# matthiasverstraete/3d_recognizer

Measured on AMD Instinct MI355X. Metric: training clouds/sec, N=40960 pts, bs=8, at 1/2/4/8 GPUs; mIoU parity, higher is better.
Workload: dtype f32 storage/accumulate, bf16x3 MFMA in the wide GEMMs

## Files before the change

### 3d_recognizer_amd/csrc/gemm.hip

```cpp
#include "rl_common.h"
#include <stdlib.h>
#include <string.h>

namespace {

typedef float f32x4 __attribute__((ext_vector_type(4)));

constexpr int GM_BM = 128;
constexpr int GM_BK = 16;
constexpr int GM_AS = 20;

struct AOperand {
    const float* A;
    long lda, a_bstride;
    int a_mode;
    RlLazy lazy;
    const float* xyz;
    long xyz_bstride;
    const int32_t* nbr_idx;
    const float* nbr_d2;
    int nbr_k;
    int n;
    int K;
    long M;
// ... 17 lines not shown
            const long R = row0 + r;
            float v[10];
#pragma unroll
            for (int c = 0; c < 10; ++c) v[c] = 0.f;
            if (R < row_limit) {
                const long p = (unsigned)R / (unsigned)a.nbr_k;
                const int b = (int)((unsigned)p / (unsigned)a.n);
                const int i = (int)(p - (long)b * a.n);
                const int j = a.nbr_idx[R];
                const float* xb = a.xyz + (long)b * a.xyz_bstride * 3;
                const float xi = xb[(long)i * 3 + 0], yi = xb[(long)i * 3 + 1], zi = xb[(long)i * 3 + 2];
                const float xj = xb[(long)j * 3 + 0], yj = xb[(long)j * 3 + 1], zj = xb[(long)j * 3 + 2];
                v[0] = xi; v[1] = yi; v[2] = zi;
                v[3] = xj; v[4] = yj; v[5] = zj;
                v[6] = xi - xj; v[7] = yi - yj; v[8] = zi - zj;
                v[9] = __fsqrt_rn(a.nbr_d2[R]);
            }
            float* dst = As + r * stride;
#pragma unroll
            for (int c = 0; c < 10; ++c) dst[c] = v[c];
            for (int c = 10; c < kw; ++c) dst[c] = 0.f;
        }
        return;
    }
    if (a.vec4) {
        const int qpr = kw >> 2;
        for (int e = tid; e < nrows * qpr; e += 256) {
            const int r = e / qpr, q = e - r * qpr;
            const long R = row0 + r;
            const int kc = k0 + q * 4;
            float4 v = make_float4(0.f, 0.f, 0.f, 0.f);
            if (R < row_limit && kc < a.K) {
                v = *reinterpret_cast<const float4*>(a.A + a_row_offset(a, R) + kc);
                if (a.lazy.scale) {
                    v.x = rl_lazy(a.lazy, v.x, kc + 0);
                    v.y = rl_lazy(a.lazy, v.y, kc + 1);
                    v.z = rl_lazy(a.lazy, v.z, kc + 2);
                    v.w = rl_lazy(a.lazy, v.w, kc + 3);
                }
            }
            *reinterpret_cast<float4*>(As + r * stride + q * 4) = v;
        }
        return;
    }
    for (int e = tid; e < nrows * kw; e += 256) {
        const int r = e / kw, c = e - r * kw;
        const long R = row0 + r;
        const int kc = k0 + c;
        float v = 0.f;
        if (R < row_limit && kc < a.K) v = rl_lazy(a.lazy, a.A[a_row_offset(a, R) + kc], kc);
        As[r * stride + c] = v;
    }
}

struct GemmParams {
    AOperand a;
    int N;
    const float* W;
    long w_ks, w_ns;
    const float* bias;
    float* Y;
    long ldy, y_bstride;
    int rows_per_batch;
    int y_contig;
    int accumulate;
    double* stats;
    const float* piv_mean;
    const float* piv_bias;
    int ksplit;
    int kchunk;
    float* kslab;
    int stat_slots;
    int gx, ny;
    const float* addend;
    float* out2;
    const int32_t* out2_index;
    long out2_bstride;
    int split_col;
    const __bf16* wsplit;
    const float* bnb_Y;
    const float* bnb_scale;
    const float* bnb_shift;
    const float* bnb_mean;
    const float* bnb_invstd;
    float bnb_neg;
    int pair_ny1;
    int N2;
    float* Y2;
    double* stats2;
    const float* piv_mean2;
    const float* piv_bias2;
    const __bf16* wsplit2;
};

__device__ __forceinline__ float stat_pivot(const GemmParams& p, int c) {
    if (!p.stats || !p.piv_mean || c >= p.N) return 0.f;
    return p.piv_mean[c] - (p.piv_bias ? p.piv_bias[c] : 0.f);
}

template <int NT>
__global__ __launch_bounds__(256) void gemm_kernel(const GemmParams p) {
    constexpr int BN = 16 * NT;
    constexpr int WS = BN + ((BN % 32 == 0) ? 16 : 0);
    __shared__ __attribute__((aligned(16))) float As[GM_BM * GM_AS];
    __shared__ float Ws[GM_BK * WS];
    __shared__ double red[4][2][BN];
// ... 57 lines not shown
                    long yoff;
                    if (p.y_contig) yoff = R * p.ldy;
                    else {
                        const int b = (int)((unsigned)R / (unsigned)p.rows_per_batch);
                        const int i = (int)(R - (long)b * p.rows_per_batch);
                        yoff = ((long)b * p.y_bstride + i) * p.ldy;
                    }
#pragma unroll
                    for (int nb = 0; nb < NT; ++nb) {
                        const int c = col0 + nb * 16 + lr;
                        if (c < N) {
                            float v = acc[rb][nb][r];
                            if (p.bias) v += p.bias[c];
                            if (p.accumulate) v += p.Y[yoff + c];
                            p.Y[yoff + c] = v;
                            const float dv = v - piv[nb];
                            ssum[nb] += dv;
                            ssq[nb] += dv * dv;
                        }
                    }
                }
            }
        }
    }
    if (p.stats) {
#pragma unroll
        for (int nb = 0; nb < NT; ++nb) {
            float s = ssum[nb], q = ssq[nb];
            s += __shfl_xor(s, 16, 64); s += __shfl_xor(s, 32, 64);
            q += __shfl_xor(q, 16, 64); q += __shfl_xor(q, 32, 64);
            if (lane < 16) {
                red[wave][0][nb * 16 + lane] = (double)s;
                red[wave][1][nb * 16 + lane] = (double)q;
            }
        }
        __syncthreads();
        if (tid < BN && col0 + tid < N) {
            const double s = red[0][0][tid] + red[1][0][tid] + red[2][0][tid] + red[3][0][tid];
            const double q = red[0][1][tid] + red[1][1][tid] + red[2][1][tid] + red[3][1][tid];
            p.stats[((long)blockIdx.x * 2 + 0) * N + col0 + tid] = s;
            p.stats[((long)blockIdx.x * 2 + 1) * N + col0 + tid] = q;
            for (long slot = blockIdx.x + gridDim.x; slot < p.stat_slots; slot += gridDim.x) {
                p.stats[(slot * 2 + 0) * N + col0 + tid] = 0.0;
                p.stats[(slot * 2 + 1) * N + col0 + tid] = 0.0;
            }
        }
    }
}

constexpr int WG_RB = 32;
constexpr int WG_T = 64;
constexpr int WG_S = 80;

struct ConcatSrc {
    const float* A2;
    const int32_t* idx;
    const float* sc2; const float* sh2;
    long a2_bstride;
    int lda2, split, act2;
    float slope2;
};

struct WgradParams {
    AOperand a;
    ConcatSrc cat;
    int N;
    const float* dY;
    long lddy, dy_bstride;
    int rows_per_batch;
    int dy_contig;
    float* slab;
    long rows_per_block;
    int has_bias;
};

__global__ __launch_bounds__(256) void wgrad_kernel(const WgradParams p) {
    __shared__ __attribute__((aligned(16))) float dYs[WG_RB * WG_S];
    __shared__ __attribute__((aligned(16))) float As[WG_RB * WG_S];
    const int tid = threadIdx.x, lane = tid & 63, wave = __builtin_amdgcn_readfirstlane(tid >> 6);
    const int lr = lane & 15, lq = lane >> 4;
    const int N = p.N, K = p.a.K;
    const int n0 = blockIdx.y * WG_T, k0 = blockIdx.z * WG_T;
    const int nvalid = min(WG_T, N - n0), kvalid = min(WG_T, K - k0);
    const int nkb = (kvalid + 15) >> 4;
    const bool wave_active = wave * 16 < nvalid;
    const long r_begin = (long)blockIdx.x * p.rows_per_block;
    const long r_end = min(p.a.M, r_begin + p.rows_per_block);

    f32x4 acc[4];
#pragma unroll
    for (int kb = 0; kb < 4; ++kb) acc[kb] = (f32x4){0.f, 0.f, 0.f, 0.f};
    float bsum = 0.f;

    for (long r0 = r_begin; r0 < r_end; r0 += WG_RB) {
        __syncthreads();
        for (int e = tid; e < WG_RB * WG_T; e += 256) {
            const int r = e >> 6, c = e & 63;
            const long R = r0 + r;
            float v = 0.f;
            if (R < r_end && c < nvalid) {
                long off;
                if (p.dy_contig) off = R * p.lddy;
                else {
                    const int b = (int)((unsigned)R / (unsigned)p.rows_per_batch);
                    const int i = (int)(R - (long)b * p.rows_per_batch);
                    off = ((long)b * p.dy_bstride + i) * p.lddy;
                }
                v = p.dY[off + n0 + c];
            }
            dYs[r * WG_S + c] = v;
        }
        stage_a(p.a, r0, WG_RB, r_end, k0, nkb * 16, As, WG_S);
        __syncthreads();
        if (p.has_bias && blockIdx.z == 0 && tid < WG_T) {
#pragma unroll 8
// ... 1138 lines not shown
        if (p.bias) {
#pragma unroll
            for (int nb = 0; nb < NT; ++nb)
                if (full || c0 + nb * 16 < N) v[nb] += *reinterpret_cast<const f32x4*>(p.bias + c0 + nb * 16);
        }
        if (p.addend) {
            const float* ad = p.addend + R * N + c0;
            f32x4 o[NT];
#pragma unroll
            for (int nb = 0; nb < NT; ++nb) o[nb] = (full || c0 + nb * 16 < N) ? *reinterpret_cast<const f32x4*>(ad + nb * 16) : (f32x4){0.f, 0.f, 0.f, 0.f};
#pragma unroll
            for (int nb = 0; nb < NT; ++nb) v[nb] += o[nb];
        }
        if (accumulate) {
            f32x4 o[NT];
#pragma unroll
            for (int nb = 0; nb < NT; ++nb) o[nb] = (full || c0 + nb * 16 < N) ? *reinterpret_cast<const f32x4*>(y + nb * 16) : (f32x4){0.f, 0.f, 0.f, 0.f};
#pragma unroll
            for (int nb = 0; nb < NT; ++nb) v[nb] += o[nb];
        }
#pragma unroll
        for (int nb = 0; nb < NT; ++nb)
            if (full || c0 + nb * 16 < N) *reinterpret_cast<f32x4*>(y + nb * 16) = v[nb];
        return;
    }
    long o2 = 0;
    if (p.out2) {
        if (p.out2_index) {
            const int b2 = (int)((unsigned)R / (unsigned)p.rows_per_batch);
            o2 = ((long)b2 * p.out2_bstride + p.out2_index[R]) * (N - p.split_col) - p.split_col;
        } else o2 = R * (N - p.split_col) - p.split_col;
    }
#pragma unroll
    for (int nb = 0; nb < NT; ++nb)
#pragma unroll
        for (int j = 0; j < 4; ++j) {
            const int c = c0 + nb * 16 + j;
            if (c < N) {
                float t = acc[nb][j];
                if (p.bias) t += p.bias[c];
                if (p.addend) t += p.addend[R * N + c];
                if (p.out2 && c >= p.split_col) {
                    if (p.out2_index) atomicAdd(p.out2 + o2 + c, t);
                    else p.out2[o2 + c] = t;
                } else {
                    if (p.accumulate) t += p.Y[yoff + c];
                    p.Y[yoff + c] = t;
                }
            }
        }
}

typedef __attribute__((address_space(3))) unsigned char rl_lds_byte;
__device__ __forceinline__ unsigned lds_address(const void* q) {
    return (unsigned)(uintptr_t)(const rl_lds_byte*)q;
}
__device__ __forceinline__ void glds16x4(const void* g0, const void* g1, const void* g2, const void* g3, unsigned l0, unsigned l1,
                                         unsigned l2, unsigned l3) {
    unsigned keep;
    asm volatile("s_mov_b32 %0, m0\n\t"
                 "s_mov_b32 m0, %5\n\ts_nop 0\n\tglobal_load_lds_dwordx4 %1, off\n\t"
                 "s_mov_b32 m0, %6\n\ts_nop 0\n\tglobal_load_lds_dwordx4 %2, off\n\t"
                 "s_mov_b32 m0, %7\n\ts_nop 0\n\tglobal_load_lds_dwordx4 %3, off\n\t"
                 "s_mov_b32 m0, %8\n\ts_nop 0\n\tglobal_load_lds_dwordx4 %4, off\n\t"
                 "s_mov_b32 m0, %0"
                 : "=&s"(keep) : "v"(g0), "v"(g1), "v"(g2), "v"(g3), "s"(l0), "s"(l1), "s"(l2), "s"(l3) : "memory");
}
__device__ __forceinline__ void glds16x2(const void* g0, const void* g1, unsigned l0, unsigned l1) {
    unsigned keep;
    asm volatile("s_mov_b32 %0, m0\n\t"
                 "s_mov_b32 m0, %3\n\ts_nop 0\n\tglobal_load_lds_dwordx4 %1, off\n\t"
                 "s_mov_b32 m0, %4\n\ts_nop 0\n\tglobal_load_lds_dwordx4 %2, off\n\t"
                 "s_mov_b32 m0, %0"
                 : "=&s"(keep) : "v"(g0), "v"(g1), "s"(l0), "s"(l1) : "memory");
}
template <int PER>
__device__ __forceinline__ void wait_vm_chunks(int n) {
    static_assert(PER == 2 || PER == 4 || PER == 8, "pieces per loader wavefront and chunk");
    if (n <= 0) asm volatile("s_waitcnt vmcnt(0)" ::: "memory");
    else if (n == 1) { if (PER == 8) asm volatile("s_waitcnt vmcnt(8)" ::: "memory"); else if (PER == 4) asm volatile("s_waitcnt vmcnt(4)" ::: "memory"); else asm volatile("s_waitcnt vmcnt(2)" ::: "memory"); }
    else if (n == 2) { if (PER == 8) asm volatile("s_waitcnt vmcnt(16)" ::: "memory"); else if (PER == 4) asm volatile("s_waitcnt vmcnt(8)" ::: "memory"); else asm volatile("s_waitcnt vmcnt(4)" ::: "memory"); }
    else if (n == 3) { if (PER == 8) asm volatile("s_waitcnt vmcnt(24)" ::: "memory"); else if (PER == 4) asm volatile("s_waitcnt vmcnt(12)" ::: "memory"); else asm volatile("s_waitcnt vmcnt(6)" ::: "memory"); }
    else { if (PER == 8) asm volatile("s_waitcnt vmcnt(32)" ::: "memory"); else if (PER == 4) asm volatile("s_waitcnt vmcnt(16)" ::: "memory"); else asm volatile("s_waitcnt vmcnt(8)" ::: "memory"); }
}
__device__ __forceinline__ void raw_barrier() {
    __builtin_amdgcn_s_barrier();
    asm volatile("" ::: "memory");
}

#ifndef W2_ABLATE
#define W2_ABLATE 0
#endif
constexpr int W2_KMAX = 1024;
constexpr int W2_THREADS = 768;
template <int TERMS, bool STATS, int AS, int WS, int BM = 128, int BN = 128>
__global__ __launch_bounds__(W2_THREADS) void wgemm2_kernel(const GemmParams pk) {
    static_assert(AS >= 3 && AS <= 6 && WS >= 2 && WS <= 6, "ring depths vs the wait table");
    static_assert((BM == 128 || BM == 64) && (BN == 128 || BN == 64), "tile shapes");
    constexpr int RB = BM / 16;
    constexpr int CG = 8 / RB;
    constexpr int NT = BN / 16 / CG;
    constexpr bool TR = !STATS;
    constexpr int A_STAGE = BM * 128;
    constexpr int W_PLANE = BN * 64;
    constexpr int W_STAGE = 2 * W_PLANE;
    constexpr int OFF_W = AS * A_STAGE, OFF_SC = OFF_W + WS * W_STAGE, OFF_RED = OFF_SC + 2 * W2_KMAX * 4;
    constexpr int TOTAL = OFF_RED + (STATS ? 8 * 2 * BN * 8 : 0);
    __shared__ __attribute__((aligned(1024))) unsigned char lds[TOTAL];
    const int tid = threadIdx.x, lane = tid & 63, wave = __builtin_amdgcn_readfirstlane(tid >> 6);
    int bx = blockIdx.x, by = 0;
    if (pk.ny > 1) {
        const int xcd = blockIdx.x & 7, s = blockIdx.x >> 3;
        by = s % pk.ny;
        bx = (s / pk.ny) * 8 + xcd;
        if (bx >= pk.gx) return;
    }
    GemmParams p = pk;
    if (pk.pair_ny1 > 0 && by >= pk.pair_ny1) {
        by -= pk.pair_ny1;
        p.N = pk.N2; p.Y = pk.Y2; p.ldy = pk.N2; p.stats = pk.stats2;
        p.piv_mean = pk.piv_mean2; p.piv_bias = pk.piv_bias2; p.wsplit = pk.wsplit2;
        p.split_col = pk.N2;
    }
    const int col0 = by * BN;
    const int K = p.a.K, N = p.N;
    const long M = p.a.M;
    const long ntiles = (M + BM - 1) / BM;
    const bool lazy = p.a.lazy.scale != nullptr;
    float* lsc = reinterpret_cast<float*>(lds + OFF_SC);
    float* lsh = lsc + W2_KMAX;
    double* red = reinterpret_cast<double*>(lds + OFF_RED);
    const unsigned lds0 = lds_address(lds);
    if (lazy) {
        for (int k = tid; k < K; k += W2_THREADS) {
            lsc[k] = p.a.lazy.scale[k];
            lsh[k] = p.a.lazy.shift[k];
        }
    }
    if constexpr (STATS) {
        for (int i = tid; i < 8 * 2 * BN; i += W2_THREADS) red[i] = 0.0;
    }
    __syncthreads();

    const int k_begin = (p.ksplit > 1) ? blockIdx.z * p.kchunk : 0;
    const int k_end = (p.ksplit > 1) ? min(K, k_begin + p.kchunk) : K;
    const int nch = (k_end - k_begin) / PG_BK;
    const bool vec_t = (N % 4 == 0) && (p.ldy % 4 == 0) && (p.split_col % 4 == 0) &&
                       (((reinterpret_cast<uintptr_t>(p.Y) | reinterpret_cast<uintptr_t>(p.out2) | reinterpret_cast<uintptr_t>(p.addend) |
                          reinterpret_cast<uintptr_t>(p.bias) | reinterpret_cast<uintptr_t>(p.kslab)) & 15) == 0);
    const int my_tiles = bx < ntiles ? (int)((ntiles - 1 - bx) / p.gx) + 1 : 0;
    const int T = my_tiles * nch;

    if (wave >= 8) __builtin_amdgcn_s_setprio(3);
    if (wave >= 10) {
        constexpr int PPP = BN / 16;
        constexpr int WI = (TERMS == 3 ? 2 : 1) * PPP / 2;
        const int lw = wave - 10;
        const __bf16* wsrc[WI];
        unsigned wdst[WI];
#pragma unroll
        for (int j = 0; j < WI; ++j) {
            const int idx = lw * WI + j, plane = idx / PPP, rg = idx % PPP;
            int col = col0 + rg * 16 + (lane >> 2);
            col = col < N ? col : N - 1;
            wsrc[j] = p.wsplit + (long)plane * N * K + (long)col * K + (lane & 3) * 8 + k_begin;
            wdst[j] = lds0 + OFF_W + plane * W_PLANE + rg * 1024;
        }
        auto issue_w = [&](int q) {
            const int k = (q % nch) * PG_BK;
            const unsigned o = __builtin_amdgcn_readfirstlane((q % WS) * W_STAGE);
            if constexpr (WI % 4 == 0) {
#pragma unroll
                for (int j = 0; j < WI; j += 4)
                    glds16x4(wsrc[j] + k, wsrc[j + 1] + k, wsrc[j + 2] + k, wsrc[j + 3] + k, wdst[j] + o, wdst[j + 1] + o, wdst[j + 2] + o,
                             wdst[j + 3] + o);
            } else {
                glds16x2(wsrc[0] + k, wsrc[1] + k, wdst[0] + o, wdst[1] + o);
            }
        };
        for (int q = 0; q < WS - 1 && q < T; ++q) issue_w(q);
        for (int q = 0; q < T; ++q) {
            wait_vm_chunks<WI>(min(WS - 2, T - 1 - q));
            raw_barrier();
            if (q + WS - 1 < T) issue_w(q + WS - 1);
        }
    } else if (wave >= 8) {
        constexpr int AI = BM / 16;
        const int lw = wave - 8;
        const float* asrc[AI];
        auto tile_sources = [&](int j) {
            const long row0 = ((long)bx + (long)j * p.gx) * BM;
#pragma unroll
            for (int i = 0; i < AI; ++i) {
                const int r = (lw * AI + i) * 8 + (lane >> 3);
                long R = row0 + r;
                R = R < M ? R : M - 1;
                asrc[i] = p.a.A + a_row_offset(p.a, R) + (((lane & 7) ^ ((r >> 1) & 7)) << 2) + k_begin;
            }
        };
        int iq = 0, ic = 0;
        auto issue_a = [&]() {
            if (ic == 0) tile_sources(iq / nch);
            const int k = ic * PG_BK;
            const unsigned l = __builtin_amdgcn_readfirstlane(lds0 + (iq % AS) * A_STAGE + lw * AI * 1024);
            glds16x4(asrc[0] + k, asrc[1] + k, asrc[2] + k, asrc[3] + k, l, l + 1024, l + 2048, l + 3072);
            if constexpr (AI == 8) glds16x4(asrc[4] + k, asrc[5] + k, asrc[6] + k, asrc[7] + k, l + 4096, l + 5120, l + 6144, l + 7168);
            ++iq;
            ic = ic + 1 == nch ? 0 : ic + 1;
        };
        while (iq < AS - 1 && iq < T) issue_a();
        for (int q = 0; q < T; ++q) {
            wait_vm_chunks<AI>(min(AS - 2, T - 1 - q));
            raw_barrier();
            if (iq < T) issue_a();
        }
    } else {
        const int lr = lane & 15, lq = lane >> 4;
        const bool relu = p.a.lazy.act == RL_ACT_RELU;
        const float nslope = p.a.lazy.act == RL_ACT_NONE ? 1.f : p.a.lazy.slope;
        const int rb = wave % RB, cg = wave / RB;
        const int cg0 = cg * NT * 16;
        const int frow = rb * 16 + lr;
        const int fsw = (frow >> 1) & 7;
        const int a_frag0 = frow * 128 + (((2 * lq) ^ fsw) << 4), a_frag1 = frow * 128 + (((2 * lq + 1) ^ fsw) << 4);
        const int w_frag = lr * 64 + lq * 16 + cg0 * 64;
        auto actf = [&](float z) {
            const float neg = relu ? 0.f : z * nslope;
            return z > 0.f ? z : neg;
        };
        f32x4 acc[NT];
#pragma unroll
        for (int nb = 0; nb < NT; ++nb) acc[nb] = (f32x4){0.f, 0.f, 0.f, 0.f};
        int c = 0;
        long tile = bx;
        for (int q = 0; q < T; ++q) {
            raw_barrier();
            const unsigned char* Ab = lds + (q % AS) * A_STAGE;
            const unsigned char* Wb = lds + OFF_W + (q % WS) * W_STAGE;
            float4 v0 = *reinterpret_cast<const float4*>(Ab + a_frag0);
            float4 v1 = *reinterpret_cast<const float4*>(Ab + a_frag1);
            if (lazy) {
                const int kk = k_begin + c * PG_BK + lq * 8;
                const float4 sc0 = *reinterpret_cast<const float4*>(lsc + kk), sc1 = *reinterpret_cast<const float4*>(lsc + kk + 4);
                const float4 sh0 = *reinterpret_cast<const float4*>(lsh + kk), sh1 = *reinterpret_cast<const float4*>(lsh + kk + 4);
                v0.x = actf(v0.x * sc0.x + sh0.x); v0.y = actf(v0.y * sc0.y + sh0.y);
                v0.z = actf(v0.z * sc0.z + sh0.z); v0.w = actf(v0.w * sc0.w + sh0.w);
                v1.x = actf(v1.x * sc1.x + sh1.x); v1.y = actf(v1.y * sc1.y + sh1.y);
                v1.z = actf(v1.z * sc1.z + sh1.z); v1.w = actf(v1.w * sc1.w + sh1.w);
            }
            bf16x4 h0, l0, h1, l1;
            split_bf16(v0, h0, l0);
            split_bf16(v1, h1, l1);
            const bf16x8 a_h = __builtin_shufflevector(h0, h1, 0, 1, 2, 3, 4, 5, 6, 7);
            const bf16x8 a_l = __builtin_shufflevector(l0, l1, 0, 1, 2, 3, 4, 5, 6, 7);
            bf16x8 b_h[NT], b_l[NT];
#pragma unroll
            for (int nb = 0; nb < NT; ++nb) {
#if W2_ABLATE == 1
                const int nbs = nb & 1;
#else
                const int nbs = nb;
#endif
                b_h[nb] = *reinterpret_cast<const bf16x8*>(Wb + w_frag + nbs * 1024);
                if constexpr (TERMS == 3) b_l[nb] = *reinterpret_cast<const bf16x8*>(Wb + W_PLANE + w_frag + nbs * 1024);
            }
#if W2_ABLATE == 3
#pragma unroll
            for (int nb = 0; nb < NT; ++nb) { acc[nb][0] += (float)b_h[nb][0] * (float)a_h[0]; acc[nb][1] += (float)b_l[nb][1] * (float)a_l[1]; }
#else
#pragma unroll
            for (int nb = 0; nb < NT; ++nb) acc[nb] = TR ? __builtin_amdgcn_mfma_f32_16x16x32_bf16(b_h[nb], a_h, acc[nb], 0, 0, 0)
                                                         : __builtin_amdgcn_mfma_f32_16x16x32_bf16(a_h, b_h[nb], acc[nb], 0, 0, 0);
            if constexpr (TERMS == 3) {
#pragma unroll
                for (int nb = 0; nb < NT; ++nb) acc[nb] = TR ? __builtin_amdgcn_mfma_f32_16x16x32_bf16(b_l[nb], a_h, acc[nb], 0, 0, 0)
                                                             : __builtin_amdgcn_mfma_f32_16x16x32_bf16(a_h, b_l[nb], acc[nb], 0, 0, 0);
#pragma unroll
                for (int nb = 0; nb < NT; ++nb) acc[nb] = TR ? __builtin_amdgcn_mfma_f32_16x16x32_bf16(b_h[nb], a_l, acc[nb], 0, 0, 0)
                                                             : __builtin_amdgcn_mfma_f32_16x16x32_bf16(a_l, b_h[nb], acc[nb], 0, 0, 0);
            }
#endif
            if (++c < nch) continue;
            c = 0;
            const long row0 = tile * BM;
            tile += p.gx;
#if W2_ABLATE == 4
#pragma unroll
            for (int nb = 0; nb < NT; ++nb) asm volatile("" :: "v"(acc[nb]));
            if (p.ksplit > 1000) {
#else
            if (p.ksplit > 1) {
#endif
                float* slab = p.kslab + (long)blockIdx.z * M * N;
                if constexpr (TR) {
// ... 17 lines not shown
                    const long R = row0 + rb * 16 + lq * 4 + r;
                    if (R < M) {
#pragma unroll
                        for (int nb = 0; nb < NT; ++nb) {
                            const int cc = col0 + cg0 + nb * 16 + lr;
                            if (cc < N) slab[R * N + cc] = acc[nb][r];
                        }
                    }
                }
                }
#if W2_ABLATE == 4
            } else if (p.ksplit > 1000) {
#else
            } else {
#endif
                float ssum[NT], ssq[NT];
#pragma unroll
                for (int nb = 0; nb < NT; ++nb) ssum[nb] = ssq[nb] = 0.f;
                if constexpr (TR) tile_rows_epilogue_t<NT>(p, acc, row0 + rb * 16, col0 + cg0, lr, lq, vec_t);
                else tile_rows_epilogue<NT, STATS>(p, acc, row0 + rb * 16, col0 + cg0, lr, lq, ssum, ssq);
                if constexpr (STATS) if (p.stats) {
#pragma unroll
                    for (int nb = 0; nb < NT; ++nb) {
                        float sv = ssum[nb], qv = ssq[nb];
                        sv += __shfl_xor(sv, 16, 64); sv += __shfl_xor(sv, 32, 64);
                        qv += __shfl_xor(qv, 16, 64); qv += __shfl_xor(qv, 32, 64);
                        if (lane < 16) {
                            red[(wave * 2 + 0) * BN + cg0 + nb * 16 + lane] += (double)sv;
                            red[(wave * 2 + 1) * BN + cg0 + nb * 16 + lane] += (double)qv;
                        }
                    }
                }
            }
#pragma unroll
            for (int nb = 0; nb < NT; ++nb) acc[nb] = (f32x4){0.f, 0.f, 0.f, 0.f};
        }
    }
    if constexpr (STATS) if (p.stats && p.ksplit <= 1) {
        __syncthreads();
        if (tid < BN && col0 + tid < N) {
            double tot_s = 0.0, tot_q = 0.0;
            for (int w = 0; w < 8; ++w) {
                tot_s += red[(w * 2 + 0) * BN + tid];
                tot_q += red[(w * 2 + 1) * BN + tid];
            }
            p.stats[((long)bx * 2 + 0) * N + col0 + tid] = tot_s;
            p.stats[((long)bx * 2 + 1) * N + col0 + tid] = tot_q;
            for (long slot = bx + p.gx; slot < p.stat_slots; slot += p.gx) {
                p.stats[(slot * 2 + 0) * N + col0 + tid] = 0.0;
                p.stats[(slot * 2 + 1) * N + col0 + tid] = 0.0;
            }
        }
    }
}

constexpr int WS_MAX = 64;
struct SplitBatch {
    rl_wsplit_item item[WS_MAX];
    int first_block[WS_MAX + 1];
    int count;
};
__global__ __launch_bounds__(256) void split_weights_kernel(const SplitBatch b) {
    int i = 0;
    while (i + 1 < b.count && (int)blockIdx.x >= b.first_block[i + 1]) ++i;
    const rl_wsplit_item& it = b.item[i];
    const unsigned K = (unsigned)it.K, N = (unsigned)it.N, kg = K >> 3;
    const unsigned e = ((unsigned)blockIdx.x - (unsigned)b.first_block[i]) * 256u + threadIdx.x;
    if (e >= N * kg) return;
    unsigned n, g;
    if (it.w_ns == 1) { g = e / N; n = e - g * N; }
    else { n = e / kg; g = e - n * kg; }
    const unsigned k0 = g * 8u;
    const float* src = it.W + (long)k0 * it.w_ks + (long)n * it.w_ns;
    float w[8];
    if (it.w_ks == 1 && ((((uintptr_t)src) & 15) == 0)) {
        const float4 a = *reinterpret_cast<const float4*>(src), c = *reinterpret_cast<const float4*>(src + 4);
        w[0] = a.x; w[1] = a.y; w[2] = a.z; w[3] = a.w; w[4] = c.x; w[5] = c.y; w[6] = c.z; w[7] = c.w;
    } else {
#pragma unroll
        for (int j = 0; j < 8; ++j) w[j] = src[(long)j * it.w_ks];
    }
    bf16x8 h, t;
#pragma unroll
    for (int j = 0; j < 8; ++j) {
        h[j] = (__bf16)w[j];
        t[j] = (__bf16)(w[j] - (float)h[j]);
    }
    __bf16* out = reinterpret_cast<__bf16*>(it.out);
    const unsigned o = n * K + k0;
    *reinterpret_cast<bf16x8*>(out + o) = h;
    *reinterpret_cast<bf16x8*>(out + (unsigned long)N * K + o) = t;
}

template <int CB>
__global__ __launch_bounds__(256) void gemm_splitk_reduce_kernel(const GemmParams p) {
    constexpr int QN = CB / 4, RP = 256 / QN;
    __shared__ float red[256][9];
    const int N = p.N;
    const long M = p.a.M;
    const int q = threadIdx.x & (QN - 1), rsub = threadIdx.x / QN;
    const int c = blockIdx.y * CB + q * 4;
    const bool cvalid = c < N;
    const long ntiles = (M + GM_BM - 1) / GM_BM;
    float4 bias = make_float4(0.f, 0.f, 0.f, 0.f);
    if (p.bias && cvalid) bias = make_float4(p.bias[c], p.bias[c + 1], p.bias[c + 2], p.bias[c + 3]);
    float acc[8] = {0.f, 0.f, 0.f, 0.f, 0.f, 0.f, 0.f, 0.f};
// ... 620 lines not shown
    } else bx = local;
    if (bx >= it.nsplit) return;
    const int by = t / (int)it.gz, bz = t - by * (int)it.gz;
    WgradParams p;
    p.a.A = it.A; p.a.lda = it.lda; p.a.a_bstride = it.a_bstride; p.a.a_mode = 0;
    p.a.lazy.scale = it.sc; p.a.lazy.shift = it.sh; p.a.lazy.act = it.act; p.a.lazy.slope = it.slope;
    p.a.xyz = nullptr; p.a.xyz_bstride = 0; p.a.nbr_idx = nullptr; p.a.nbr_d2 = nullptr; p.a.nbr_k = 0;
    p.a.n = it.n; p.a.K = it.K; p.a.M = it.M; p.a.contig = it.a_contig; p.a.vec4 = 1; p.a.vec4p = 1;
    p.N = it.N; p.dY = it.dY; p.lddy = it.lddy; p.dy_bstride = it.dy_bstride; p.rows_per_batch = it.rows_per_batch;
    p.dy_contig = it.dy_contig; p.slab = it.slab; p.rows_per_block = it.rows_per_block; p.has_bias = it.has_bias;
    p.cat = ConcatSrc{};
    if (it.cat) p.cat = b.cat[it.cat - 1];
    pwgrad128w_body<TERMS, false>(p, bx, by, bz);
}

__global__ __launch_bounds__(256) void swgrad_batch_kernel(const WgradBatch b) {
    __shared__ float red[4 * 4 * 4 * 64 + 8 * 64];
    int i = 0;
    while (i + 1 < b.count && (int)blockIdx.x >= b.item[i + 1].first_block) ++i;
    const WBItem& it = b.item[i];
    WgradParams p;
    p.a.A = it.A; p.a.lda = it.lda; p.a.a_bstride = it.a_bstride; p.a.a_mode = 0;
    p.a.lazy.scale = it.sc; p.a.lazy.shift = it.sh; p.a.lazy.act = it.act; p.a.lazy.slope = it.slope;
    p.a.xyz = nullptr; p.a.xyz_bstride = 0; p.a.nbr_idx = nullptr; p.a.nbr_d2 = nullptr; p.a.nbr_k = 0;
    p.a.n = it.n; p.a.K = it.K; p.a.M = it.M; p.a.contig = it.a_contig; p.a.vec4 = 0; p.a.vec4p = 0;
    p.N = it.N; p.dY = it.dY; p.lddy = it.lddy; p.dy_bstride = it.dy_bstride; p.rows_per_batch = it.rows_per_batch;
    p.dy_contig = it.dy_contig; p.slab = it.slab; p.rows_per_block = it.rows_per_block; p.has_bias = it.has_bias;
    p.cat = ConcatSrc{};
    const int bx = (int)blockIdx.x - it.first_block;
    if (bx >= it.nsplit) return;
    switch (it.gy) {
        case swgrad_body_index(1, 1): swgrad_body<1, 1>(p, bx, red); break;
        case swgrad_body_index(1, 2): swgrad_body<1, 2>(p, bx, red); break;
        case swgrad_body_index(1, 4): swgrad_body<1, 4>(p, bx, red); break;
        case swgrad_body_index(1, 8): swgrad_body<1, 8>(p, bx, red); break;
        case swgrad_body_index(2, 1): swgrad_body<2, 1>(p, bx, red); break;
        case swgrad_body_index(2, 2): swgrad_body<2, 2>(p, bx, red); break;
        case swgrad_body_index(2, 4): swgrad_body<2, 4>(p, bx, red); break;
        case swgrad_body_index(4, 1): swgrad_body<4, 1>(p, bx, red); break;
        case swgrad_body_index(4, 2): swgrad_body<4, 2>(p, bx, red); break;
        default: swgrad_body<4, 4>(p, bx, red); break;
    }
}

inline bool pwgrad_ok(const WgradParams& p) {
    if (p.a.a_mode != 0 || !p.a.vec4) return false;
    if ((p.N % 4) || (p.lddy % 4) || (((uintptr_t)p.dY) & 15)) return false;
    if (p.a.lazy.scale && ((((uintptr_t)p.a.lazy.scale) | ((uintptr_t)p.a.lazy.shift)) & 15)) return false;
    return true;
}


typedef void (*GemmFn)(const GemmParams);
typedef void (*WgradFn)(const WgradParams);
enum GemmKernel { GK_NONE, GK_SGEMM, GK_PGEMM, GK_WGEMM, GK_WGEMM2, GK_GEMM };

struct GemmFacts {
    long M; int N, K;
    bool streamable;
    bool pgemm, wgemm, wgemm2;
    bool split, stats, bnb;
    int64_t kslab_floats;
};

struct GemmPlan {
    GemmKernel kernel;
    GemmFn fn;
    int threads; dim3 grid;
    WidePlan wide;
    int gx, ny, ksplit, kchunk;
    GemmFn reduce;
    dim3 reduce_grid;
    const char* name;
    const char* refusal;
};

template <int KC, bool BNB>
GemmFn sgemm_fn(int N) {
    if constexpr (KC == 1 && !BNB) if (N > 64) return sgemm_kernel<1, 8>;
    return N <= 16 ? sgemm_kernel<KC, 1, BNB> : N <= 32 ? sgemm_kernel<KC, 2, BNB> : sgemm_kernel<KC, 4, BNB>;
}
template <int NT>
GemmFn pgemm_fn(int terms) { return terms == 0 ? pgemm_kernel<NT, 0> : terms == 1 ? pgemm_kernel<NT, 1> : pgemm_kernel<NT, 3>; }
template <int TERMS, bool STATS>
GemmFn wide_inst(bool dma, WidePlan w) {
    if (!dma) return wgemm_kernel<TERMS, STATS>;
    return w.bm == 128 ? wgemm2_kernel<TERMS, STATS, W2_AS, W2_WS, 128, 128>
         : w.bn == 128 ? wgemm2_kernel<TERMS, STATS, W2_AS, W2_WS, 64, 128> : wgemm2_kernel<TERMS, STATS, W2_AS, W2_WS, 64, 64>;
}
inline GemmFn wide_fn(bool stats, bool dma, WidePlan w) {
    if (wide_gemm_terms() == 1) return stats ? wide_inst<1, true>(dma, w) : wide_inst<1, false>(dma, w);
    return stats ? wide_inst<3, true>(dma, w) : wide_inst<3, false>(dma, w);
}

inline dim3 xcd_grid(int gx, int ny, int z) { return dim3(ny > 1 ? (unsigned)(8 * rl_cdiv(gx, 8) * ny) : (unsigned)gx, 1, z); }

inline void persistent_grid(GemmPlan& pl, long M, int ny, int z) {
    int cap = cu_count() / ny / 8 * 8;
    if (cap < 8) cap = 8;
    pl.gx = rl_cdiv(M, pl.wide.bm);
    if (pl.gx > cap) pl.gx = cap;
    pl.ny = ny;
    pl.grid = xcd_grid(pl.gx, ny, z);
}

inline void plan_wide(GemmPlan& pl, const GemmFacts& f, int z, bool splitk) {
    const bool dma = f.wgemm2;
    pl.fn = wide_fn(f.stats && pl.ksplit <= 1, dma, pl.wide);
    pl.kernel = dma ? GK_WGEMM2 : GK_WGEMM;
    pl.threads = dma ? W2_THREADS : 512;
    if (dma) persistent_grid(pl, f.M, rl_cdiv(f.N, pl.wide.bn), z);
    else     pl.grid = xcd_grid(pl.gx, pl.ny, z);
    pl.name = dma ? (splitk ? "wgemm2_kernel+splitk" : "wgemm2_kernel") : (splitk ? "wgemm_kernel+splitk" : "wgemm_kernel");
}

GemmPlan plan_gemm(const GemmFacts& f) {
    const int N = f.N, K = f.K, nt = N <= 16 ? 1 : N <= 32 ? 2 : N <= 64 ? 4 : 8;
    GemmPlan pl{};
    pl.threads = 256; pl.ksplit = 1;
    pl.gx = rl_row_blocks_host(f.M, GM_BM);
    pl.ny = N > 64 ? rl_cdiv(N, 128) : 1;
    if (f.split && K <= 64 && N <= 64) { pl.refusal = "rl_gemm: split-scatter epilogue needs K or N > 64"; return pl; }
    if (f.split && !f.pgemm) { pl.refusal = "rl_gemm: split-scatter epilogue needs the LDS-tiled kernel (aligned operands, K % 4 == 0)"; return pl; }
    const bool streams = !f.split && f.streamable && stream_ok(N, K);
    if (!f.split && f.bnb && !(streams && N <= 64)) {
        pl.refusal = "rl_gemm: the BatchNorm-backward sums are a by-product of the streaming kernel only (K, N <= 64; ask rl_gemm_streams)";
        return pl;
    }
    if (streams) {
        int sg = pl.gx;
        if ((long)K * N >= 2048) sg = sg > 512 ? 512 : (sg > 256 ? 256 : sg);
        if (g_sgemm_grid_div > 1) sg = sg / g_sgemm_grid_div > 0 ? sg / g_sgemm_grid_div : 1;
        if (f.bnb) pl.fn = K <= 16 ? sgemm_fn<1, true>(N) : K <= 32 ? sgemm_fn<2, true>(N) : sgemm_fn<4, true>(N);
        else       pl.fn = K <= 16 ? sgemm_fn<1, false>(N) : K <= 32 ? sgemm_fn<2, false>(N) : sgemm_fn<4, false>(N);
        pl.kernel = GK_SGEMM;
        pl.grid = dim3(sg);
        pl.name = "sgemm_kernel";
        return pl;
    }
    if (f.pgemm) pl.wide = wide_plan(f.M, N, K, N > 64 && f.wgemm && f.wgemm2);
    const int terms = wide_gemm_terms();
    if (!f.split && f.pgemm && N > 64 && pl.wide.ksplit > 1 && f.kslab_floats >= (int64_t)pl.wide.ksplit * f.M * N) {
        pl.kchunk = ((K + pl.wide.ksplit - 1) / pl.wide.ksplit + 31) / 32 * 32;
        pl.ksplit = (K + pl.kchunk - 1) / pl.kchunk;
        const bool cb64 = (long)pl.gx * rl_cdiv(N, 64) >= 256;
        pl.reduce = cb64 ? gemm_splitk_reduce_kernel<64> : gemm_splitk_reduce_kernel<16>;
        pl.reduce_grid = dim3(pl.gx, rl_cdiv(N, cb64 ? 64 : 16));
        if (f.wgemm) {
            plan_wide(pl, f, pl.ksplit, true);
        } else {
            pl.kernel = GK_PGEMM;
            pl.fn = pgemm_fn<8>(terms);
            pl.grid = xcd_grid(pl.gx, pl.ny, pl.ksplit);
            pl.name = "pgemm_kernel<8>+splitk";
        }
    } else if (!f.split && f.pgemm && N > 16 && N <= 64 && wgemm_small_tiles() && f.wgemm && f.wgemm2) {
        pl.wide = WidePlan{64, 64, 1};
        plan_wide(pl, f, 1, false);
    } else if (!f.pgemm) {
        pl.kernel = GK_GEMM;
        pl.fn = nt == 1 ? gemm_kernel<1> : nt == 2 ? gemm_kernel<2> : nt == 4 ? gemm_kernel<4> : gemm_kernel<8>;
        pl.grid = dim3(pl.gx, pl.ny);
        pl.name = "gemm_kernel";
    } else if (N > 64 && f.wgemm) {
        plan_wide(pl, f, 1, false);
    } else {
        pl.kernel = GK_PGEMM;
        pl.fn = nt == 1 ? pgemm_fn<1>(terms) : nt == 2 ? pgemm_fn<2>(terms) : nt == 4 ? pgemm_fn<4>(terms) : pgemm_fn<8>(terms);
        pl.grid = xcd_grid(pl.gx, pl.ny, 1);
        pl.name = N > 64 ? "pgemm_kernel<8>" : f.split ? "pgemm_kernel" : nt == 1 ? "pgemm_kernel<1>" : nt == 2 ? "pgemm_kernel<2>" : "pgemm_kernel<4>";
    }
    return pl;
}

inline GemmFacts aligned_facts(long M, int N, int K, bool dma) {
    return GemmFacts{M, N, K, true, true, wide_gemm_terms() != 0 && K % 8 == 0,
                     dma && wgemm_staging() == 1 && K % PG_BK == 0 && K <= W2_KMAX, false, true, false, 0};
}

int launch_gemm(const GemmPlan& pl, hipStream_t st, GemmParams p, const char* who) {
    p.gx = pl.gx; p.ny = pl.ny; p.ksplit = pl.ksplit; p.kchunk = pl.kchunk;
    hipLaunchKernelGGL(pl.fn, pl.grid, dim3(pl.threads), 0, st, p);
    rl_note_kernel(pl.name);
    RL_LAUNCH_CHECK(who);
    if (!pl.reduce) return RL_OK;
    hipLaunchKernelGGL(pl.reduce, pl.reduce_grid, dim3(256), 0, st, p);
    RL_LAUNCH_CHECK("rl_gemm(split-K reduce)");
    return RL_OK;
}

struct WgradPlan {
    WgradFn fn;
    int threads; dim3 grid;
    int nsplit; long rows_per_block;
    int batch;
    int body;
    const char* name;
    const char* refusal;
};

template <int KT>
WgradFn swgrad_fn(int N) {
    if constexpr (KT == 1) if (N > 64) return swgrad_kernel<1, 8>;
    return N <= 16 ? swgrad_kernel<KT, 1> : N <= 32 ? swgrad_kernel<KT, 2> : swgrad_kernel<KT, 4>;
}

WgradPlan plan_wgrad(long M, int N, int K, int a_mode, bool pwgrad, bool rows_bf16, int cat_split = 0) {
    if (cat_split != 0) {
        WgradPlan pl = plan_wgrad(M, N, K, a_mode, pwgrad, rows_bf16);
        const bool w = pl.fn == (WgradFn)pwgrad128w_kernel<1> || pl.fn == (WgradFn)pwgrad128w_kernel<3>;
        if (!(w && !rows_bf16 && K == 2 * cat_split && cat_split % 16 == 0)) {
            pl.fn = nullptr;
            pl.batch = 0;
            pl.refusal = "rl_wgrad: a concat-gather A operand (a2_split) needs the wide (128 x 128 tile) kernel outside the fp32 "
                         "arithmetic mode, fp32 rows, K == 2 * a2_split and a2_split % 16 == 0";
        }
        return pl;
    }
    WgradPlan pl{};
    pl.threads = 256;
    const int terms = wide_gemm_terms();
    if (stream_ok(N, K)) {
        swgrad_split(M, &pl.nsplit, &pl.rows_per_block);
        if (!rows_bf16) pl.fn = K <= 16 ? swgrad_fn<1>(N) : K <= 32 ? swgrad_fn<2>(N) : swgrad_fn<4>(N);
        pl.refusal = "rl_wgrad: bf16 rows are supported by the wide weight-gradient kernel only";
        pl.grid = dim3(pl.nsplit);
        pl.batch = a_mode == 0 && !rows_bf16 ? 2 : 0;
        pl.body = swgrad_body_index(K <= 16 ? 1 : K <= 32 ? 2 : 4, N <= 16 ? 1 : N <= 32 ? 2 : N <= 64 ? 4 : 8);
        pl.name = "swgrad_kernel";
        return pl;
    }
    wgrad_split(M, N, K, &pl.nsplit, &pl.rows_per_block);
    const int T = pwgrad ? wgrad_tile(N, K) : WG_T;
    const bool wide = pwgrad && T == 128;
    pl.grid = dim3(pl.nsplit, rl_cdiv(N, T), rl_cdiv(K, T));
    if (rows_bf16)  pl.fn = wide && terms != 0 ? pwgrad128w_kernel<1, true> : nullptr;
    else if (wide)  pl.fn = terms == 0 ? pwgrad128_kernel : terms == 1 ? pwgrad128w_kernel<1> : pwgrad128w_kernel<3>;
    else            pl.fn = pwgrad ? pwgrad_kernel : wgrad_kernel;
    pl.threads = wide && terms != 0 ? 512 : 256;
    pl.refusal = "rl_wgrad: bf16 rows are supported by the wide (128 x 128 tile) weight-gradient kernel only";
    pl.batch = !rows_bf16 && wide && terms != 0 && rl_cdiv(N, 128) < 65536 && rl_cdiv(K, 128) < 65536 ? 1 : 0;
    pl.name = wide ? (terms != 0 ? "pwgrad128w_kernel" : "pwgrad128_kernel") : pwgrad ? "pwgrad_kernel" : "wgrad_kernel";
    return pl;
}

void launch_wgrad_batch(int batch, long blocks, hipStream_t st, const WgradBatch& b) {
    if (batch == 2)                   hipLaunchKernelGGL(swgrad_batch_kernel, dim3((unsigned)blocks), dim3(256), 0, st, b);
    else if (wide_gemm_terms() == 1)  hipLaunchKernelGGL(pwgrad128w_batch_kernel<1>, dim3((unsigned)blocks), dim3(512), 0, st, b);
    else                              hipLaunchKernelGGL(pwgrad128w_batch_kernel<3>, dim3((unsigned)blocks), dim3(512), 0, st, b);
}

}

int rl_wide_terms() { return wide_gemm_terms(); }

extern "C" int rl_set_wide_gemm(const char* mode) {
    const int t = parse_wide(mode);
    RL_REQUIRE(mode != nullptr && t >= 0, RL_ERR_ARGS, "rl_set_wide_gemm: mode must be \"fp32\", \"bf16x3\" or \"bf16\"");
    g_wide_terms = t;
    return RL_OK;
}
extern "C" int rl_set_wgemm_staging(const char* how) {
    RL_REQUIRE(how != nullptr && (!strcmp(how, "registers") || !strcmp(how, "dma")), RL_ERR_ARGS,
               "rl_set_wgemm_staging: \"registers\" or \"dma\"");
    g_wgemm_staging = !strcmp(how, "dma");
    return RL_OK;
}
extern "C" int rl_set_wgemm_tile(const char* how) {
    RL_REQUIRE(how && (!strcmp(how, "auto") || !strcmp(how, "128") || !strcmp(how, "64x128") || !strcmp(how, "64x64")), RL_ERR_ARGS,
               "rl_set_wgemm_tile: expected auto | 128 | 64x128 | 64x64");
    g_wgemm_force = !strcmp(how, "64x128") ? 1 : !strcmp(how, "64x64") ? 2 : 0;
    g_wgemm_small = strcmp(how, "128") ? 1 : 0;
    return RL_OK;
}
extern "C" int rl_set_gemm_ksplit(int enable) {
    g_gemm_no_ksplit = enable ? 0 : 1;
    return RL_OK;
}
extern "C" int rl_set_sgemm_grid_div(int div) {
    RL_REQUIRE(div >= 1 && div <= 64, RL_ERR_ARGS, "rl_set_sgemm_grid_div: 1 .. 64");
    g_sgemm_grid_div = div;
    return RL_OK;
}
extern "C" const char* rl_get_wide_gemm(void) {
    const int t = wide_gemm_terms();
    return t == 0 ? "fp32" : t == 1 ? "bf16" : "bf16x3";
}

extern "C" int rl_gemm(const rl_gemm_desc* d, void* stream) {
    RL_REQUIRE(d != nullptr, RL_ERR_ARGS, "rl_gemm: null descriptor");
    GemmParams p{};
    int rc = fill_a(&p.a, "rl_gemm", d->A, d->lda, d->a_bstride, d->a_mode, d->in_act, d->in_slope,
                    d->in_scale, d->in_shift, d->xyz, d->xyz_bstride, d->nbr_idx, d->nbr_d2, d->nbr_k,
                    d->B, d->n, d->K);
    if (rc) return rc;
    RL_REQUIRE(d->N > 0 && d->W && d->Y && d->ldy > 0, RL_ERR_ARGS, "rl_gemm: bad W/Y");
    p.N = d->N; p.W = d->W; p.w_ks = d->w_ks; p.w_ns = d->w_ns; p.bias = d->bias;
    p.Y = d->Y; p.ldy = d->ldy; p.y_bstride = d->y_bstride;
    p.rows_per_batch = (d->a_mode == 1) ? d->n * d->nbr_k : d->n;
    RL_REQUIRE(d->y_bstride >= p.rows_per_batch, RL_ERR_ARGS, "rl_gemm: y_bstride smaller than rows per cloud");
    p.y_contig = (d->y_bstride == p.rows_per_batch);
    p.accumulate = d->accumulate; p.stats = d->stats;
    p.piv_mean = d->stats ? d->stats_pivot_mean : nullptr; p.piv_bias = d->stats ? d->stats_pivot_bias : nullptr;
    p.addend = d->addend; p.out2 = d->out2; p.out2_index = d->out2_index; p.out2_bstride = d->out2_bstride;
    RL_REQUIRE(!d->out2_index || rl_float_atomics_allowed(), RL_ERR_UNSUPPORTED,
               "rl_gemm: out2_index scatters with fp32 atomics (order-dependent); the deterministic path is a dense out2 + "
               "rl_segment_sum_rows (set RL_ALLOW_FLOAT_ATOMICS=1 to use it anyway)");
    p.split_col = d->out2 ? d->split_col : d->N;
    p.wsplit = reinterpret_cast<const __bf16*>(d->W_split);
    const bool split = d->addend != nullptr || d->out2 != nullptr;
    if (split) {
        RL_REQUIRE(!d->out2 || (d->split_col > 0 && d->split_col < d->N && (!d->out2_index || d->out2_bstride > 0)), RL_ERR_ARGS,
                   "rl_gemm: bad split-scatter fields");
        RL_REQUIRE(d->ldy >= (d->out2 ? d->split_col : d->N), RL_ERR_ARGS, "rl_gemm: ldy smaller than the columns stored to Y");
        RL_REQUIRE(d->stats == nullptr, RL_ERR_UNSUPPORTED, "rl_gemm: split-scatter epilogue has no statistics");
    } else {
        RL_REQUIRE(d->ldy >= d->N, RL_ERR_ARGS, "rl_gemm: bad W/Y");
    }
    p.stat_slots = (int)rl_gemm_stat_slots(p.a.M, d->N, d->K);
    const GemmPlan pl = plan_gemm(GemmFacts{p.a.M, d->N, d->K, p.a.a_mode == 0 && p.a.vec4p, pgemm_ok(p), wgemm_ok(p), wgemm2_usable(p),
                                            split, d->stats != nullptr, d->bnb_Y != nullptr, d->kslab ? d->kslab_floats : 0});
    RL_REQUIRE(pl.kernel != GK_NONE, RL_ERR_UNSUPPORTED, "%s", pl.refusal);
    if (!split && d->bnb_Y) {
        RL_REQUIRE(d->stats && d->bnb_scale && d->bnb_shift && d->bnb_mean && d->bnb_invstd && !d->stats_pivot_mean, RL_ERR_ARGS,
                   "rl_gemm: bnb_Y needs stats, the layer's scale / shift / mean / invstd and no pivot");
        p.bnb_Y = d->bnb_Y; p.bnb_scale = d->bnb_scale; p.bnb_shift = d->bnb_shift; p.bnb_mean = d->bnb_mean; p.bnb_invstd = d->bnb_invstd;
        p.bnb_neg = d->bnb_act == RL_ACT_RELU ? 0.f : (d->bnb_act == RL_ACT_LRELU ? d->bnb_slope : 1.f);
        p.piv_mean = p.piv_bias = nullptr;
    }
    p.kslab = pl.reduce ? d->kslab : nullptr;
    return launch_gemm(pl, (hipStream_t)stream, p, "rl_gemm");
}

extern "C" int rl_gemm_streams(const rl_gemm_desc* d) {
    if (!d) return 0;
    const bool vec4p = (d->lda % 4 == 0) && ((d->K + 3) / 4 * 4 <= d->lda) && (((uintptr_t)d->A & 15) == 0);
    const GemmFacts f{(long)d->B * d->n, d->N, d->K, d->a_mode == 0 && vec4p, false, false, false, d->addend || d->out2, false, false, 0};
    return (plan_gemm(f).kernel == GK_SGEMM && d->N <= 64) ? 1 : 0;
}

static bool gemm_pair_fits(const rl_gemm_desc* a, const rl_gemm_desc* b) {
    if (!a || !b) return false;
    if (a->A != b->A || a->lda != b->lda || a->a_bstride != b->a_bstride || a->a_mode != 0 || b->a_mode != 0) return false;
    if (a->B != b->B || a->n != b->n || a->K != b->K) return false;
    if (a->in_scale != b->in_scale || a->in_shift != b->in_shift || a->in_act != b->in_act || a->in_slope != b->in_slope) return false;
    if (!a->W_split || !b->W_split || wide_gemm_terms() == 0 || wgemm_staging() != 1) return false;
    if (a->K % PG_BK || a->K > W2_KMAX || a->N <= 0 || b->N <= 0) return false;
    if ((a->K <= 64 && a->N <= 64) || (b->K <= 64 && b->N <= 64)) return false;
    if (a->bias || b->bias || a->accumulate || b->accumulate || a->addend || b->addend || a->out2 || b->out2) return false;
    if ((a->stats == nullptr) != (b->stats == nullptr)) return false;
    if (a->ldy != a->N || b->ldy != b->N || a->y_bstride != a->n || b->y_bstride != b->n || !a->Y || !b->Y) return false;
    if ((((uintptr_t)a->A | (uintptr_t)(a->lda * 4) | (uintptr_t)a->W_split | (uintptr_t)b->W_split | (uintptr_t)a->Y | (uintptr_t)b->Y) & 15) != 0)
        return false;
    if (a->N % 4 || b->N % 4) return false;
    return true;
}
extern "C" int rl_gemm_pair_supported(const rl_gemm_desc* a, const rl_gemm_desc* b) { return gemm_pair_fits(a, b) ? 1 : 0; }
extern "C" int rl_gemm_pair(const rl_gemm_desc* a, const rl_gemm_desc* b, void* stream) {
    RL_REQUIRE(gemm_pair_fits(a, b), RL_ERR_UNSUPPORTED,
               "rl_gemm_pair: needs one plain A' (K %% 32 == 0, K <= 1024) for both, pre-split weights in a bf16 arithmetic mode, the "
               "dense outputs, statistics for both or none, no bias / accumulate / split epilogue");
    GemmParams p{};
    int rc = fill_a(&p.a, "rl_gemm_pair", a->A, a->lda, a->a_bstride, 0, a->in_act, a->in_slope, a->in_scale, a->in_shift,
                    nullptr, 0, nullptr, nullptr, 0, a->B, a->n, a->K);
    if (rc) return rc;
    p.N = a->N; p.W = a->W; p.w_ks = a->w_ks; p.w_ns = a->w_ns; p.bias = nullptr;
    p.Y = a->Y; p.ldy = a->ldy; p.y_bstride = a->y_bstride; p.rows_per_batch = a->n; p.y_contig = 1;
    p.accumulate = 0; p.stats = a->stats;
    p.piv_mean = a->stats ? a->stats_pivot_mean : nullptr; p.piv_bias = a->stats ? a->stats_pivot_bias : nullptr;
    p.split_col = a->N; p.wsplit = reinterpret_cast<const __bf16*>(a->W_split);
    p.stat_slots = rl_row_blocks_host(p.a.M, GM_BM);
    p.N2 = b->N; p.Y2 = b->Y; p.stats2 = b->stats; p.wsplit2 = reinterpret_cast<const __bf16*>(b->W_split);
    p.piv_mean2 = b->stats ? b->stats_pivot_mean : nullptr; p.piv_bias2 = b->stats ? b->stats_pivot_bias : nullptr;
    p.pair_ny1 = rl_cdiv(a->N, 128);
    RL_REQUIRE(wgemm2_usable(p), RL_ERR_UNSUPPORTED, "rl_gemm_pair: the LDS-DMA kernel does not take this operand");
    GemmPlan pl{};
    pl.kernel = GK_WGEMM2; pl.wide = WidePlan{128, 128, 1}; pl.threads = W2_THREADS; pl.ksplit = 1; pl.name = "wgemm2_kernel";
    pl.fn = wide_fn(p.stats != nullptr, true, pl.wide);
    persistent_grid(pl, p.a.M, p.pair_ny1 + rl_cdiv(b->N, 128), 1);
    return launch_gemm(pl, (hipStream_t)stream, p, "rl_gemm_pair");
}

extern "C" int rl_split_weights(const rl_wsplit_item* items, int count, void* stream) {
    RL_REQUIRE(items != nullptr && count >= 0, RL_ERR_ARGS, "rl_split_weights: bad arguments");
    hipStream_t st = (hipStream_t)stream;
    for (int base = 0; base < count; base += WS_MAX) {
        SplitBatch b;
        b.count = count - base < WS_MAX ? count - base : WS_MAX;
        long blocks = 0;
        for (int i = 0; i < b.count; ++i) {
// ... 197 lines not shown
```

### 3d_recognizer_amd/csrc/rl_common.h

```cpp
#pragma once
#include <hip/hip_runtime.h>
#include <stdarg.h>
#include <stdint.h>
#include <stdio.h>

#include "../../include/rl_randlanet.h"

void rl_set_error(const char* fmt, ...);
void rl_note_kernel(const char* name);

#define RL_REQUIRE(cond, code, ...)      \
    do {                                 \
        if (!(cond)) {                   \
            rl_set_error(__VA_ARGS__);   \
            return (code);               \
        }                                \
    } while (0)

#define RL_LAUNCH_CHECK(name)                                                        \
    do {                                                                             \
        hipError_t e_ = hipGetLastError();                                           \
        if (e_ != hipSuccess) {                                                      \
            rl_set_error("%s: launch failed: %s", name, hipGetErrorString(e_));      \
            return RL_ERR_LAUNCH;                                                    \
// ... 33 lines not shown
        at += al256(bytes);
        return off;
    }
};

template <class T>
static inline T* rl_at(const void* ws, size_t off) { return (T*)((char*)ws + off); }

static inline int rl_ws_check(const char* who, const void* ws, int64_t ws_bytes, int64_t need) {
    RL_REQUIRE(ws_bytes >= need, RL_ERR_ARGS, "%s: workspace of %lld bytes, %lld needed", who, (long long)ws_bytes,
               (long long)need);
    RL_REQUIRE(ws, RL_ERR_ARGS, "%s: null pointer", who);
    RL_REQUIRE(((uintptr_t)ws & 255) == 0, RL_ERR_ARGS, "%s: workspace not 256-byte aligned", who);
    return RL_OK;
}

static inline int rl_bits_of(int64_t x) {
    int b = 0;
    while (x > 0) ++b, x >>= 1;
    return b < 1 ? 1 : b;
}

#define RL_ACT_NONE 0
#define RL_ACT_RELU 1
#define RL_ACT_LRELU 2

__device__ __forceinline__ float rl_act(float z, int act, float slope) {
    if (act == RL_ACT_RELU) return z > 0.f ? z : 0.f;
    if (act == RL_ACT_LRELU) return z > 0.f ? z : z * slope;
    return z;
}
__device__ __forceinline__ float rl_act_grad(float z, int act, float slope) {
    if (act == RL_ACT_RELU) return z > 0.f ? 1.f : 0.f;
    if (act == RL_ACT_LRELU) return z > 0.f ? 1.f : slope;
    return 1.f;
}

struct RlLazy {
    const float* scale;
    const float* shift;
    int act;
    float slope;
};
__device__ __forceinline__ float rl_lazy(const RlLazy& t, float raw, int c) {
    if (t.scale == nullptr) return raw;
    return rl_act(raw * t.scale[c] + t.shift[c], t.act, t.slope);
}

typedef float rl_f32x4 __attribute__((ext_vector_type(4)));
__device__ __forceinline__ float rl_eff_slope(const RlLazy& t) {
    if (t.scale == nullptr || t.act == RL_ACT_NONE) return 1.f;
    return t.act == RL_ACT_RELU ? 0.f : t.slope;
}
__device__ __forceinline__ rl_f32x4 rl_fold_act4(const rl_f32x4 raw, const rl_f32x4 scale, const rl_f32x4 shift, const float e) {
    const rl_f32x4 z = raw * scale + shift;
    const rl_f32x4 ev = {e, e, e, e};
    return __builtin_elementwise_max(z, z * ev);
}

typedef __bf16 rl_bf16x4 __attribute__((ext_vector_type(4)));
template <bool BF>
__device__ __forceinline__ float rl_ldx(const float* p, long i) {
    if constexpr (BF) return (float)reinterpret_cast<const __bf16*>(p)[i];
    else return p[i];
}
template <bool BF>
__device__ __forceinline__ void rl_stx(float* p, long i, float v) {
    if constexpr (BF) reinterpret_cast<__bf16*>(p)[i] = (__bf16)v;
    else p[i] = v;
}
template <bool BF>
__device__ __forceinline__ float4 rl_ldx4(const float* p, long i) {
    if constexpr (BF) {
        const rl_bf16x4 h = *reinterpret_cast<const rl_bf16x4*>(reinterpret_cast<const __bf16*>(p) + i);
        return make_float4((float)h[0], (float)h[1], (float)h[2], (float)h[3]);
    } else return *reinterpret_cast<const float4*>(p + i);
}
template <bool BF>
__device__ __forceinline__ void rl_stx4(float* p, long i, const float4 v) {
    if constexpr (BF) {
        rl_bf16x4 h;
        h[0] = (__bf16)v.x; h[1] = (__bf16)v.y; h[2] = (__bf16)v.z; h[3] = (__bf16)v.w;
        *reinterpret_cast<rl_bf16x4*>(reinterpret_cast<__bf16*>(p) + i) = h;
    } else *reinterpret_cast<float4*>(p + i) = v;
}
template <bool BF>
__device__ __forceinline__ void rl_stx_nt(float* p, long i, float v) {
    if constexpr (BF) __builtin_nontemporal_store((__bf16)v, reinterpret_cast<__bf16*>(p) + i);
    else __builtin_nontemporal_store(v, p + i);
}
template <bool BF>
__device__ __forceinline__ void rl_stx4_nt(float* p, long i, const float4 v) {
    typedef float rl_f32x4 __attribute__((ext_vector_type(4)));
    if constexpr (BF) {
        rl_bf16x4 h;
        h[0] = (__bf16)v.x; h[1] = (__bf16)v.y; h[2] = (__bf16)v.z; h[3] = (__bf16)v.w;
        __builtin_nontemporal_store(h, reinterpret_cast<rl_bf16x4*>(reinterpret_cast<__bf16*>(p) + i));
    } else {
        const rl_f32x4 w = {v.x, v.y, v.z, v.w};
        __builtin_nontemporal_store(w, reinterpret_cast<rl_f32x4*>(p + i));
    }
}
__device__ __forceinline__ float4 rl_ld4(const float* p, long i, int bf) { return bf ? rl_ldx4<true>(p, i) : rl_ldx4<false>(p, i); }
__device__ __forceinline__ float rl_ld1(const float* p, long i, int bf) { return bf ? rl_ldx<true>(p, i) : rl_ldx<false>(p, i); }
__device__ __forceinline__ void rl_st4(float* p, long i, const float4 v, int bf) {
    if (bf) rl_stx4<true>(p, i, v);
// ... 18 lines not shown
```

### 3d_recognizer_amd/csrc/rows.hip

```cpp
#include "rl_common.h"

namespace {

struct RowsParams {
    const float* src;
    long lds, src_bstride;
    float* dst;
    long ldd;
    long rows, rows_per_batch;
    int C;
    const int32_t* i32;
    const int64_t* i64;
    int shared;
    int accumulate;
    RlLazy lazy;
};

template <typename I>
__device__ __forceinline__ long src_row(const RowsParams& p, I r) {
    const I b = r / (I)p.rows_per_batch;
    const I i = r - b * (I)p.rows_per_batch;
    long j = i;
    if (p.i32) j = p.shared ? p.i32[i] : p.i32[r];
    else if (p.i64) j = p.shared ? p.i64[i] : p.i64[r];
    return (long)b * p.src_bstride + j;
}

template <typename I>
__device__ __forceinline__ void copy_rows_quads(const RowsParams& p) {
    const int cpr = p.C / 4;
    const long total = p.rows * cpr;
    {
        typedef float v4f __attribute__((ext_vector_type(4)));
        const bool lazy = p.lazy.scale != nullptr;
        const float es = (!lazy || p.lazy.act == RL_ACT_NONE) ? 1.f : (p.lazy.act == RL_ACT_RELU ? 0.f : p.lazy.slope);
        const long stride = (long)gridDim.x * 256;
        for (long e0 = (long)blockIdx.x * 256 + threadIdx.x; e0 < total; e0 += 4 * stride) {
            long so[4], dofs[4];
            int cc[4];
            bool ok[4];
#pragma unroll
            for (int u = 0; u < 4; ++u) {
                const long e = e0 + u * stride;
                ok[u] = e < total;
                const I ee = (I)(ok[u] ? e : e0);
                const I r = ee / (I)cpr;
                cc[u] = (int)(ee - r * (I)cpr) * 4;
                so[u] = src_row<I>(p, r) * p.lds + cc[u];
                dofs[u] = (long)r * p.ldd + cc[u];
            }
            v4f v[4], o[4];
#pragma unroll
// ... 27 lines not shown
    if constexpr (VEC == 4) {
        copy_rows_quads<I>(p);
    } else {
        for (long e = (long)blockIdx.x * 256 + threadIdx.x; e < total; e += (long)gridDim.x * 256) {
            const I r = (I)e / (I)cpr;
            const int c = (int)((I)e - r * (I)cpr) * VEC;
            const long so = src_row<I>(p, r) * p.lds + c;
            const long dofs = (long)r * p.ldd + c;
            float v = rl_lazy(p.lazy, p.src[so], c);
            if (p.accumulate) v += p.dst[dofs];
            p.dst[dofs] = v;
        }
    }
}

struct RowsPair {
    RowsParams p[2];
};
__global__ __launch_bounds__(256) void copy_rows_pair_kernel(const RowsPair q) {
    const RowsParams& p = q.p[blockIdx.y];
    copy_rows_quads<uint32_t>(p);
}

template <typename I>
__global__ __launch_bounds__(256) void scatter_add_rows_kernel(const RowsParams p) {
    const long total = p.rows * p.C;
    for (long e = (long)blockIdx.x * 256 + threadIdx.x; e < total; e += (long)gridDim.x * 256) {
        const I r = (I)e / (I)p.C;
        const int c = (int)((I)e - r * (I)p.C);
        const long drow = src_row<I>(p, r);
        atomicAdd(p.dst + drow * p.ldd + c, p.src[(long)r * p.lds + c]);
    }
}

int fill(RowsParams* p, const rl_rows_desc* d, const char* who) {
    RL_REQUIRE(d && d->src && d->dst && d->rows >= 0 && d->rows_per_batch > 0 && d->C > 0, RL_ERR_ARGS, "%s: bad descriptor", who);
    RL_REQUIRE(!(d->index32 && d->index64), RL_ERR_ARGS, "%s: give index32 or index64, not both", who);
    RL_REQUIRE((d->scale == nullptr) == (d->shift == nullptr), RL_ERR_ARGS, "%s: scale/shift must come together", who);
    p->src = d->src; p->lds = d->lds; p->src_bstride = d->src_bstride; p->dst = d->dst; p->ldd = d->ldd;
    p->rows = d->rows; p->rows_per_batch = d->rows_per_batch; p->C = d->C; p->i32 = d->index32;
    p->i64 = d->index64; p->shared = d->index_shared; p->accumulate = d->accumulate;
    p->lazy.scale = d->scale; p->lazy.shift = d->shift; p->lazy.act = d->act; p->lazy.slope = d->slope;
    return RL_OK;
}

inline bool fits32(long elements) { return elements < (1l << 32); }

int grid_for(long work) {
    long g = (work + 255) / 256;
    if (g < 1) g = 1;
    return (int)(g < 4096 ? g : 4096);
}

template <typename I>
__global__ __launch_bounds__(256) void attpool_fwd16_kernel(const float* __restrict__ X, const float* __restrict__ S,
                                                            long P, int C, float* __restrict__ Pout) {
    const long total = P * C;
    for (long e = (long)blockIdx.x * 256 + threadIdx.x; e < total; e += (long)gridDim.x * 256) {
        const long pt = (long)((I)e / (I)C);
        const int c = (int)(e - pt * C);
        const float* s = S + pt * 16 * C + c;
        const float* x = X + pt * 16 * C + c;
        float sv[16], xv[16];
#pragma unroll
        for (int k = 0; k < 16; ++k) sv[k] = s[(long)k * C];
#pragma unroll
        for (int k = 0; k < 16; ++k) xv[k] = x[(long)k * C];
        float m = sv[0];
#pragma unroll
        for (int k = 1; k < 16; ++k) m = fmaxf(m, sv[k]);
        float den = 0.f, num = 0.f;
#pragma unroll
        for (int k = 0; k < 16; ++k) {
            const float w = expf(sv[k] - m);
            den += w;
            num += w * xv[k];
        }
        Pout[e] = num / den;
    }
}
template <typename I>
__global__ __launch_bounds__(256) void attpool_bwd16_kernel(const float* __restrict__ X, const float* __restrict__ S,
                                                            const float* __restrict__ Pout, const float* __restrict__ dP,
                                                            long P, int C, float* __restrict__ dS, float* __restrict__ dXa) {
    const long total = P * C;
    for (long e = (long)blockIdx.x * 256 + threadIdx.x; e < total; e += (long)gridDim.x * 256) {
        const long pt = (long)((I)e / (I)C);
        const int c = (int)(e - pt * C);
        const long base = pt * 16 * C + c;
        float sv[16], xv[16];
#pragma unroll
        for (int k = 0; k < 16; ++k) sv[k] = S[base + (long)k * C];
#pragma unroll
        for (int k = 0; k < 16; ++k) xv[k] = X[base + (long)k * C];
        const float g = dP[e], po = Pout[e];
        float m = sv[0];
#pragma unroll
        for (int k = 1; k < 16; ++k) m = fmaxf(m, sv[k]);
        float den = 0.f;
#pragma unroll
        for (int k = 0; k < 16; ++k) {
            sv[k] = expf(sv[k] - m);
            den += sv[k];
        }
        const float inv = 1.f / den;
#pragma unroll
        for (int k = 0; k < 16; ++k) {
            const long o = base + (long)k * C;
            const float a = sv[k] * inv;
            dXa[o] = g * a;
            dS[o] = a * g * (xv[k] - po);
        }
    }
}

template <typename I>
__global__ __launch_bounds__(256) void attpool_fwd_kernel(const float* __restrict__ X, const float* __restrict__ S,
                                                          long P, int K, int C, float* __restrict__ Pout) {
    const long total = P * C;
    for (long e = (long)blockIdx.x * 256 + threadIdx.x; e < total; e += (long)gridDim.x * 256) {
        const long pt = (long)((I)e / (I)C);
        const int c = (int)(e - pt * C);
        const float* s = S + pt * K * C + c;
        const float* x = X + pt * K * C + c;
        float m = s[0];
        for (int k = 1; k < K; ++k) m = fmaxf(m, s[(long)k * C]);
        float den = 0.f, num = 0.f;
        for (int k = 0; k < K; ++k) {
            const float w = expf(s[(long)k * C] - m);
            den += w;
            num += w * x[(long)k * C];
        }
        Pout[e] = num / den;
    }
}

template <typename I>
__global__ __launch_bounds__(256) void attpool_bwd_kernel(const float* __restrict__ X, const float* __restrict__ S,
                                                          const float* __restrict__ Pout, const float* __restrict__ dP,
                                                          long P, int K, int C, float* __restrict__ dS,
                                                          float* __restrict__ dXa) {
    const long total = P * C;
    for (long e = (long)blockIdx.x * 256 + threadIdx.x; e < total; e += (long)gridDim.x * 256) {
        const long pt = (long)((I)e / (I)C);
        const int c = (int)(e - pt * C);
        const long base = pt * K * C + c;
        float m = S[base];
// ... 191 lines not shown
    rl_note_kernel("copy_rows_kernel");
    RL_LAUNCH_CHECK("rl_copy_rows");
    return RL_OK;
}

extern "C" int rl_copy_rows_pair(const rl_rows_desc* d0, const rl_rows_desc* d1, void* stream) {
    RowsPair q;
    int rc = fill(&q.p[0], d0, "rl_copy_rows_pair");
    if (rc) return rc;
    rc = fill(&q.p[1], d1, "rl_copy_rows_pair");
    if (rc) return rc;
    bool ok = true;
    long quads = 0;
    for (const RowsParams& p : q.p) {
        ok = ok && p.rows > 0 && (p.C % 4 == 0) && (p.lds % 4 == 0) && (p.ldd % 4 == 0) && (((uintptr_t)p.src & 15) == 0) &&
             (((uintptr_t)p.dst & 15) == 0) && (!p.lazy.scale || ((((uintptr_t)p.lazy.scale) | ((uintptr_t)p.lazy.shift)) & 15) == 0) &&
             fits32(p.rows * p.C) && fits32(p.rows_per_batch);
        const long q4 = (p.rows * (p.C / 4) + 3) / 4;
        quads = q4 > quads ? q4 : quads;
    }
    if (!ok) {
        rc = rl_copy_rows(d0, stream);
        return rc ? rc : rl_copy_rows(d1, stream);
    }
    hipLaunchKernelGGL(copy_rows_pair_kernel, dim3(grid_for(quads), 2), dim3(256), 0, (hipStream_t)stream, q);
    rl_note_kernel("copy_rows_pair_kernel");
    RL_LAUNCH_CHECK("rl_copy_rows_pair");
    return RL_OK;
}

extern "C" int rl_scatter_add_rows(const rl_rows_desc* d, void* stream) {
    RowsParams p;
    int rc = fill(&p, d, "rl_scatter_add_rows");
    if (rc) return rc;
    RL_REQUIRE(p.i32 || p.i64, RL_ERR_ARGS, "rl_scatter_add_rows: needs an index");
    RL_REQUIRE(rl_float_atomics_allowed(), RL_ERR_UNSUPPORTED,
               "rl_scatter_add_rows: fp32 atomics are order-dependent; the deterministic path is rl_csr_build + rl_segment_sum_rows "
               "(set RL_ALLOW_FLOAT_ATOMICS=1 to use this entry point anyway)");
    RL_REQUIRE(p.lazy.scale == nullptr, RL_ERR_ARGS, "rl_scatter_add_rows: no lazy transform here");
    if (p.rows == 0) return RL_OK;
    if (fits32(p.rows * p.C) && fits32(p.rows_per_batch))
        hipLaunchKernelGGL(scatter_add_rows_kernel<uint32_t>, dim3(grid_for(p.rows * p.C)), dim3(256), 0, (hipStream_t)stream, p);
    else
        hipLaunchKernelGGL(scatter_add_rows_kernel<int64_t>, dim3(grid_for(p.rows * p.C)), dim3(256), 0, (hipStream_t)stream, p);
    rl_note_kernel("scatter_add_rows_kernel");
    RL_LAUNCH_CHECK("rl_scatter_add_rows");
    return RL_OK;
}

extern "C" int rl_attpool_fwd(const float* X, const float* S, int64_t P, int K, int C, float* Pout, void* stream) {
    RL_REQUIRE(X && S && Pout && P >= 0 && K > 0 && C > 0, RL_ERR_ARGS, "rl_attpool_fwd: bad arguments");
    if (P == 0) return RL_OK;
    if (fits32(P * C)) {
        if (K == 16) hipLaunchKernelGGL(attpool_fwd16_kernel<uint32_t>, dim3(grid_for(P * C)), dim3(256), 0, (hipStream_t)stream, X, S, (long)P, C, Pout);
        else hipLaunchKernelGGL(attpool_fwd_kernel<uint32_t>, dim3(grid_for(P * C)), dim3(256), 0, (hipStream_t)stream, X, S, (long)P, K, C, Pout);
    } else {
        hipLaunchKernelGGL(attpool_fwd_kernel<int64_t>, dim3(grid_for(P * C)), dim3(256), 0, (hipStream_t)stream, X, S, (long)P, K, C, Pout);
    }
    rl_note_kernel("attpool_fwd_kernel");
    RL_LAUNCH_CHECK("rl_attpool_fwd");
    return RL_OK;
}

extern "C" int rl_attpool_bwd(const float* X, const float* S, const float* Pout, const float* dP, int64_t P, int K,
                              int C, float* dS, float* dXa, void* stream) {
    RL_REQUIRE(X && S && Pout && dP && dS && dXa && P >= 0 && K > 0 && C > 0, RL_ERR_ARGS, "rl_attpool_bwd: bad arguments");
    if (P == 0) return RL_OK;
    if (fits32(P * C) && K == 16)
        hipLaunchKernelGGL(attpool_bwd16_kernel<uint32_t>, dim3(grid_for(P * C)), dim3(256), 0, (hipStream_t)stream, X, S, Pout, dP,
                           (long)P, C, dS, dXa);
    else if (fits32(P * C))
        hipLaunchKernelGGL(attpool_bwd_kernel<uint32_t>, dim3(grid_for(P * C)), dim3(256), 0, (hipStream_t)stream, X, S, Pout, dP,
                           (long)P, K, C, dS, dXa);
    else
        hipLaunchKernelGGL(attpool_bwd_kernel<int64_t>, dim3(grid_for(P * C)), dim3(256), 0, (hipStream_t)stream, X, S, Pout, dP,
                           (long)P, K, C, dS, dXa);
    rl_note_kernel("attpool_bwd_kernel");
    RL_LAUNCH_CHECK("rl_attpool_bwd");
    return RL_OK;
}

extern "C" int rl_add_act_fwd(const float* Y1, const float* s1, const float* b1, const float* Y2, const float* s2,
                              const float* b2, int64_t rows, int C, float slope, float* O, void* stream) {
    RL_REQUIRE(Y1 && s1 && b1 && Y2 && s2 && b2 && O && rows >= 0 && C > 0, RL_ERR_ARGS, "rl_add_act_fwd: bad arguments");
    if (rows == 0) return RL_OK;
    const bool vec = C % 4 == 0 && ((((uintptr_t)Y1) | ((uintptr_t)Y2) | ((uintptr_t)O) | ((uintptr_t)s1) | ((uintptr_t)b1) |
                                      ((uintptr_t)s2) | ((uintptr_t)b2)) & 15) == 0;
    if (vec) {
        const long quads = (long)rows * (C / 4);
        hipLaunchKernelGGL(add_act_fwd_vec_kernel, dim3(grid_for((quads + 1) / 2)), dim3(256), 0, (hipStream_t)stream, Y1, s1, b1, Y2,
                           s2, b2, quads, C, slope, O);
    } else if (fits32(rows * C))
        hipLaunchKernelGGL(add_act_fwd_kernel<uint32_t>, dim3(grid_for(rows * C)), dim3(256), 0, (hipStream_t)stream, Y1, s1, b1, Y2,
                           s2, b2, (long)rows * C, C, slope, O);
    else
        hipLaunchKernelGGL(add_act_fwd_kernel<int64_t>, dim3(grid_for(rows * C)), dim3(256), 0, (hipStream_t)stream, Y1, s1, b1, Y2,
                           s2, b2, (long)rows * C, C, slope, O);
    rl_note_kernel("add_act_fwd_kernel");
    RL_LAUNCH_CHECK("rl_add_act_fwd");
    return RL_OK;
}

extern "C" int rl_add_act_bwd(float* G, const float* O, int64_t rows, int C, float slope, void* stream) {
    RL_REQUIRE(G && O && rows >= 0 && C > 0, RL_ERR_ARGS, "rl_add_act_bwd: bad arguments");
    if (rows == 0) return RL_OK;
    hipLaunchKernelGGL(add_act_bwd_kernel, dim3(grid_for(rows * C)), dim3(256), 0, (hipStream_t)stream, G, O,
                       (long)rows * C, slope);
    rl_note_kernel("add_act_bwd_kernel");
    RL_LAUNCH_CHECK("rl_add_act_bwd");
    return RL_OK;
}

static int rpe_build_impl(const float* xyz, int64_t xyz_bstride, const int32_t* nbr_idx, const float* nbr_d2, int B,
                          int n, int k, float* out, int is_distance, void* stream) {
    RL_REQUIRE(xyz && nbr_idx && nbr_d2 && out && B > 0 && n > 0 && k > 0 && xyz_bstride >= n, RL_ERR_ARGS,
               "rl_rpe_build: bad arguments");
    RL_REQUIRE((((uintptr_t)out) & 15) == 0, RL_ERR_ARGS, "rl_rpe_build: out must be 16-byte aligned");
    const long rows = (long)B * n * k;
    RL_REQUIRE(rows < (1l << 31), RL_ERR_ARGS, "rl_rpe_build: too many rows");
    hipLaunchKernelGGL(rpe_build_kernel, dim3(grid_for(rows)), dim3(256), 0, (hipStream_t)stream, xyz, (long)xyz_bstride,
                       nbr_idx, nbr_d2, (unsigned)n, (unsigned)k, rows, out, is_distance);
    rl_note_kernel("rpe_build_kernel");
    RL_LAUNCH_CHECK("rl_rpe_build");
    return RL_OK;
}

extern "C" int rl_rpe_build(const float* xyz, int64_t xyz_bstride, const int32_t* nbr_idx, const float* nbr_d2, int B,
                            int n, int k, float* out, void* stream) {
    return rpe_build_impl(xyz, xyz_bstride, nbr_idx, nbr_d2, B, n, k, out, 0, stream);
}

extern "C" int rl_rpe_build_dist(const float* xyz, int64_t xyz_bstride, const int32_t* nbr_idx, const float* nbr_dist, int B,
                                 int n, int k, float* out, void* stream) {
// ... 99 lines not shown
```

### 3d_recognizer_amd/randlanet/_engine.py

```python
from dataclasses import dataclass, field
from typing import ClassVar, Dict, List, Optional

import torch

from . import _hip as H
from . import _ops as ops
from ._ops import Lazy, Rpe

BN_EPS = 1e-6
BN_MOMENTUM = 0.99
BN_PIVOT = True
BAND_SORT_MIN_POINTS = 4096


@dataclass(slots=True, eq=False)
class _Record:
    kind: ClassVar[str] = ""
    level: int = field(default=-1, init=False)


@dataclass(slots=True, eq=False)
class LinearRec(_Record):
    kind: ClassVar[str] = "linear"
    a: object
    out: Lazy
    wname: str
    bname: Optional[str]
    ks: int
    ns: int
    a_grad: bool
    last_consumer_of_input: int


@dataclass(slots=True, eq=False)
class PoolRec(_Record):
    kind: ClassVar[str] = "pool"
    name: str
    u: Lazy
    g: Lazy
    csr: object
    X: torch.Tensor
    S: torch.Tensor
    pooled: Lazy
    n: int
    d: int


@dataclass(slots=True, eq=False)
class PoolFusedRec(_Record):
    kind: ClassVar[str] = "pool_fused"
    name: str
    u: object
    g: Lazy
    csr: object
    idx: torch.Tensor
    pooled: Lazy
    n: int
    d: int
    stage: int


@dataclass(slots=True, eq=False)
class AddActRec(_Record):
    kind: ClassVar[str] = "add_act"
    m2: Lazy
    sc: Lazy
    O: Lazy


@dataclass(slots=True, eq=False)
class InterpConcatRec(_Record):
    kind: ClassVar[str] = "interp_concat"
    prev: Lazy
    skip: Lazy
    csr: object
    catl: Lazy


@dataclass(slots=True, eq=False)
class HeadRec(_Record):
    kind: ClassVar[str] = "head"
    x: Lazy
    head: object
    drop: tuple


@dataclass(slots=True, eq=False)
class DropoutPhiloxRec(_Record):
    kind: ClassVar[str] = "dropout_philox"
    src: Lazy
    dropped: Lazy
    key: torch.Tensor
    p_drop: float
    seed: int
# ... 158 lines not shown
                     wsplit=ctx.wsplit, pivot=(piv, self.P[bname] if fold else None) if piv is not None else None)
        rpb = a.n * a.K if isinstance(a, Rpe) else a.n
        out = Lazy(Y, a.B, rpb, rpb, n_out)
        if bn:
            self._bn(ctx, out, stats, bn, act, slope, folded_bias=self.P[bname] if fold else None,
                     nslots=ops.gemm_stat_slots(out.rows, n_out, K) if stats is not None else None)
        else:
            assert act == H.ACT_NONE
        ctx.record(LinearRec(a, out, wname, bname, ks, ns, a_grad, last_consumer_of_input))
        return out

    def _mlp_pair(self, ctx, a: Lazy, first: tuple, second: tuple, first_is_last_consumer: int = 0):
        specs, metas = [], []
        for name, n_out, act, slope in (first, second):
            wname, bname, bn = f"{name}.conv.weight", f"{name}.conv.bias", f"{name}.batch_norm"
            W = self._w2(wname)
            ks, ns = ops.weight_strides(W, False, a.C, n_out)
            stats = ops.new_stats(W.device, n_out) if ctx.training else None
            piv = self._pivot(ctx, bn) if stats is not None else None
            specs.append((W, ks, ns, n_out, stats, (piv, self.P[bname]) if piv is not None else None))
            metas.append((wname, bname, bn, n_out, act, slope, ks, ns, stats))
        res = ops.gemm_pair(a, specs[0], specs[1], ctx.wsplit)
        if res is None:
            return self._mlp(ctx, a, *first, last_consumer_of_input=first_is_last_consumer), self._mlp(ctx, a, *second)
        outs = []
        for Y, (wname, bname, bn, n_out, act, slope, ks, ns, stats), last in zip(res, metas, (first_is_last_consumer, 0)):
            out = Lazy(Y, a.B, a.n, a.n, n_out)
            self._bn(ctx, out, stats, bn, act, slope, folded_bias=self.P[bname],
                     nslots=H.row_blocks(out.rows, 128) if stats is not None else None)
            ctx.record(LinearRec(a, out, wname, bname, ks, ns, True, last))
            outs.append(out)
        return outs[0], outs[1]

    def _mlp(self, ctx, a, name: str, n_out: int, act: int = H.ACT_NONE, slope: float = 0.0, *, transposed=False,
             bn=True, a_grad=True, last_consumer_of_input: int = 0) -> Lazy:
        return self._linear(ctx, a, f"{name}.conv.weight", f"{name}.conv.bias", n_out, transposed=transposed,
                            bn=f"{name}.batch_norm" if bn else None, act=act, slope=slope, a_grad=a_grad,
                            last_consumer_of_input=last_consumer_of_input)

    def _pool(self, ctx, name: str, u, g: Lazy, idx: torch.Tensor, csr, n: int, d: int, n_out: int, stage: int = 0,
              next_stats: bool = False) -> Lazy:
        B, K, h = u.B, self.K, d // 2
        rows = B * n * K
        Ws = self.P[f"{name}.score_fn.0.weight"]
        if ops.pool_supported(d, K):
            if next_stats:
                res, st2, ns2 = ops.pool_fwd(u, g, idx, Ws, n, d, stage, next_stats=True)
                ctx.next_stats = (st2, ns2)
            else:
                res = ops.pool_fwd(u, g, idx, Ws, n, d, stage)
            pooled = ops.plain(res, B, n)
            ctx.record(PoolFusedRec(name, u, g, csr, idx, pooled, n, d, stage))
            return self._mlp(ctx, pooled, f"{name}.mlp", n_out, H.ACT_RELU)
        X = torch.empty((rows, d), dtype=torch.float32, device=u.raw.device)
        ops.copy_rows_pair(((u.raw, (0, h), n * K, X, (0, h), rows, n * K), dict(lazy=u)),
                           ((g.raw, (0, h), g.bstride, X, (h, h), rows, n * K), dict(index=idx, lazy=g)))
        S = ops.gemm(ops.plain(X, B, n * K), Ws, 1, d, d, None, wsplit=ctx.wsplit)
        Pt = ops.attpool_fwd(X, S, B * n, K)
        pooled = ops.plain(Pt, B, n)
        ctx.record(PoolRec(name, u, g, csr, X, S, pooled, n, d))
        return self._mlp(ctx, pooled, f"{name}.mlp", n_out, H.ACT_RELU)

    def _virtual_bn(self, ctx: Context, vr, stage: int, bn_name: str, stats=None, nslots: int = 1) -> Lazy:
        if ctx.training and stats is None:
            stats, nslots = ops.rpe_stats(vr, stage)
        scale, shift, mean, invstd = self._fold(ctx, bn_name, stats, vr.rows, vr.h, None, nslots)
        rec = Lazy(vr.d2, vr.B, vr.n * 16, vr.n * 16, vr.h, scale, shift, H.ACT_RELU, 0.0, mean, invstd, bn_name)
        return rec

    def _lfa(self, ctx, l: int, xin: Lazy, xyz: torch.Tensor, n: int, d: int, idx, d2, csr=None) -> Lazy:
        e = f"encoder.{l}"
        B, K, h = xin.B, self.K, d // 2
        ctx.keep += [idx, d2]
        ctx.bn_defer = [] if self.sync is None else None
        f0, sc = self._mlp_pair(ctx, xin, (f"{e}.mlp1", h, H.ACT_LRELU, 0.2), (f"{e}.shortcut", 2 * d, H.ACT_NONE, 0.0),
                                first_is_last_consumer=2 if l == 0 else 0)
        if ops.virtual_rpe_supported(d, K, B * n, n):
            vr = ops.VirtualRpe(ctx.xyz4 if ctx.xyz4 is not None else xyz, idx, d2, B, n, h, self.P[f"{e}.mlp_rpe1.conv.weight"], self.P[f"{e}.mlp_rpe1.conv.bias"],
                                self.P[f"{e}.mlp_rpe2.conv.weight"], self.P[f"{e}.mlp_rpe2.conv.bias"])
            vr.piv1, vr.piv2 = self._pivot(ctx, f"{e}.mlp_rpe1.batch_norm"), self._pivot(ctx, f"{e}.mlp_rpe2.batch_norm")
            vr.bn1 = self._virtual_bn(ctx, vr, 1, f"{e}.mlp_rpe1.batch_norm")
            ops.bn_finalize_flush(ctx.bn_defer)
            q1 = self._pool(ctx, f"{e}.pool1", vr, f0, idx, csr, n, d, h, stage=1, next_stats=ctx.training)
            vr.bn2 = self._virtual_bn(ctx, vr, 2, f"{e}.mlp_rpe2.batch_norm", *ctx.next_stats)
            ctx.next_stats = (None, 1)
            ops.bn_finalize_flush(ctx.bn_defer)
            ctx.bn_defer = None
            q2 = self._pool(ctx, f"{e}.pool2", vr, q1, idx, csr, n, d, d, stage=2)
        else:
            rpe = Rpe(xyz, idx, d2, B, n, K)
            if h <= 128:
                rpe = ops.rpe_build(rpe)
            u1 = self._mlp(ctx, rpe, f"{e}.mlp_rpe1", h, H.ACT_RELU, a_grad=False)
            ops.bn_finalize_flush(ctx.bn_defer)
            q1 = self._pool(ctx, f"{e}.pool1", u1, f0, idx, csr, n, d, h)
            u2 = self._mlp(ctx, u1, f"{e}.mlp_rpe2", h, H.ACT_RELU)
            ops.bn_finalize_flush(ctx.bn_defer)
            ctx.bn_defer = None
            q2 = self._pool(ctx, f"{e}.pool2", u2, q1, idx, csr, n, d, d)
        m2 = self._mlp(ctx, q2, f"{e}.mlp2", 2 * d, last_consumer_of_input=1)
        O = ops.plain(ops.add_act_fwd(m2, sc, 0.01), B, n)
        ctx.record(AddActRec(m2, sc, O))
        return O

    def _wide_weight_uses(self, training: bool):
        uses = []
        for name, W in self.P.items():
            if not name.endswith(("conv.weight", "score_fn.0.weight")) or W.dim() < 2:
                continue
            a, b = int(W.shape[0]), int(W.shape[1])
            if max(a, b) <= 64:
                if name.endswith(".mlp1.conv.weight") and b % 32 == 0 and b > 64:
                    sc = self.P.get(name.replace(".mlp1.", ".shortcut."))
                    if sc is not None and int(sc.shape[0]) > 64:
# ... 261 lines not shown
            st.bn_pre[id(r.x.raw)] = pre

    def _bwd_dropout_philox(self, st: _Backward, r: DropoutPhiloxRec):
        G = st.arrived(r.dropped).buf
        ops.dropout_bwd(G, r.key, r.seed, r.p_drop, r.first_row)
        st.put(r.src, G)

    def _bwd_dropout(self, st: _Backward, r: DropoutRec):
        G = st.arrived(r.dropped).buf
        ops.scale_mask(G, r.mask, r.scale)
        st.put(r.src, G)

    def _bwd_pool_virtual(self, st: _Backward, r: PoolFusedRec):
        name, vr, g, n, d, stage, grads = r.name, r.u, r.g, r.n, r.d, r.stage, st.grads
        h = d // 2
        e = name.rsplit(".", 1)[0]
        GP = st.arrived(r.pooled).buf
        key = ("vgu", id(vr))
        if stage == 2:
            GU = torch.empty((vr.rows, h), dtype=ops.row_dtype(), device=GP.device)
            first = True
        else:
            GU, first = st.slots.pop(key).buf, False
        gg = st.slot(g)
        nslots = H.lib().rl_pool_bwd_slots(vr.B * n, d)
        bstats = torch.empty((nslots, 2, h), dtype=torch.float64, device=GP.device)
        DG = ops.pool_bwd(vr, g, r.idx, self.P[f"{name}.score_fn.0.weight"], n, d, GP, GU, not first,
                          grads[f"{name}.score_fn.0.weight"], pending=st.pending, stage=stage, bn_bwd_stats=bstats)
        ops.segment_sum_rows(DG, (0, h), n * self.K, r.csr, gg.buf, g.bstride, accumulate=gg.written)
        gg.written = True
        layer = f"{e}.mlp_rpe{stage}"
        queue = st.fin_queue if self.sync is None else None
        coef = ops.rpe_bn_backward(vr, stage, GU, grads[f"{layer}.batch_norm.weight"], grads[f"{layer}.batch_norm.bias"],
                                   sync=self.sync, stats=bstats, nslots=nslots, queue=queue)
        GU1 = torch.empty_like(GU) if stage == 2 else None

        def finish():
            with ops.level(r.level):
                ops.rpe_wgrad(vr, stage, GU, coef, grads[f"{layer}.conv.weight"], grads[f"{layer}.conv.bias"], st.pending, GU1)
        if queue is not None:
            st.rpe_after.append(finish)
        else:
            finish()
        if stage == 2:
            st.slots[key] = GradSlot(GU1, True)

    def _bwd_pool(self, st: _Backward, r: PoolRec):
        name, u, g, csr, X, S, pooled, n, d, grads = r.name, r.u, r.g, r.csr, r.X, r.S, r.pooled, r.n, r.d, st.grads
        B, K, h = u.B, self.K, d // 2
        rows = B * n * K
        GP = st.arrived(pooled).buf
        dS, dX = ops.attpool_bwd(X, S, pooled.raw, GP, B * n, K)
        Ws = self.P[f"{name}.score_fn.0.weight"]
        ops.wgrad(ops.plain(X, B, n * K), dS, n * K, d, grads[f"{name}.score_fn.0.weight"], 1, d, None, pending=st.pending,
                  batch=st.wbatch)
        gu = st.slot(u)
        gg = st.slot(g)
        if d <= 64:
            ops.gemm(ops.plain(dS, B, n * K), Ws, d, 1, d, None, out=dX, out_bstride=n * K, accumulate=True,
                     wsplit=st.wsplit)
            ops.copy_rows(dX, (0, h), n * K, gu.buf, (0, h), rows, n * K, accumulate=gu.written)
            ops.segment_sum_rows(dX, (h, h), n * K, csr, gg.buf, g.bstride, accumulate=gg.written)
        else:
            DG = torch.empty((rows, h), dtype=torch.float32, device=dX.device)
            ops.gemm(ops.plain(dS, B, n * K), Ws, d, 1, d, None, out=gu.buf, out_bstride=n * K, accumulate=gu.written,
                     addend=dX, out2=DG, split_col=h, wsplit=st.wsplit)
            ops.segment_sum_rows(DG, (0, h), n * K, csr, gg.buf, g.bstride, accumulate=gg.written)
        gu.written = gg.written = True

    _BWD = {"linear": _bwd_linear, "pool": _bwd_pool, "pool_fused": _bwd_pool_fused, "add_act": _bwd_add_act,
            "interp_concat": _bwd_interp_concat, "head": _bwd_head, "dropout_philox": _bwd_dropout_philox,
            "dropout": _bwd_dropout}
```

### 3d_recognizer_amd/randlanet/_hip.py

```python
import ctypes as C
import os
from typing import Optional

import torch

_LIB: Optional[C.CDLL] = None
_LIB_PATH = os.path.join(os.path.dirname(os.path.dirname(os.path.abspath(__file__))), "csrc",
                         "librandla_hip.so")
_LIB_PATH = os.environ.get("RL_HIP_LIB", _LIB_PATH)

ABI_VERSION = 110
MAX_SLOTS = 1024
KNN_MAX_K = 64
ACT_NONE, ACT_RELU, ACT_LRELU = 0, 1, 2

ERR_ARGS, ERR_FEW_SUPPORT, ERR_LAUNCH, ERR_UNSUPPORTED = -1, -2, -3, -4


class HipKernelError(RuntimeError):
    pass


class GemmDesc(C.Structure):
    _fields_ = [
        ("A", C.c_void_p), ("lda", C.c_int64), ("a_bstride", C.c_int64),
        ("a_mode", C.c_int32), ("in_act", C.c_int32), ("in_slope", C.c_float),
        ("in_scale", C.c_void_p), ("in_shift", C.c_void_p),
        ("xyz", C.c_void_p), ("xyz_bstride", C.c_int64),
        ("nbr_idx", C.c_void_p), ("nbr_d2", C.c_void_p), ("nbr_k", C.c_int32),
        ("B", C.c_int32), ("n", C.c_int32), ("N", C.c_int32), ("K", C.c_int32),
        ("W", C.c_void_p), ("w_ks", C.c_int64), ("w_ns", C.c_int64),
        ("bias", C.c_void_p),
        ("Y", C.c_void_p), ("ldy", C.c_int64), ("y_bstride", C.c_int64),
        ("accumulate", C.c_int32),
        ("stats", C.c_void_p),
        ("kslab", C.c_void_p), ("kslab_floats", C.c_int64),
        ("addend", C.c_void_p), ("out2", C.c_void_p), ("out2_index", C.c_void_p), ("out2_bstride", C.c_int64),
        ("split_col", C.c_int32),
        ("W_split", C.c_void_p),
        ("stats_pivot_mean", C.c_void_p), ("stats_pivot_bias", C.c_void_p),
        ("bnb_Y", C.c_void_p), ("bnb_scale", C.c_void_p), ("bnb_shift", C.c_void_p), ("bnb_mean", C.c_void_p),
        ("bnb_invstd", C.c_void_p), ("bnb_act", C.c_int32), ("bnb_slope", C.c_float),
    ]


class WsplitItem(C.Structure):
    _fields_ = [("W", C.c_void_p), ("w_ks", C.c_int64), ("w_ns", C.c_int64), ("K", C.c_int32), ("N", C.c_int32),
                ("out", C.c_void_p)]


class WgradDesc(C.Structure):
    _fields_ = [
        ("A", C.c_void_p), ("lda", C.c_int64), ("a_bstride", C.c_int64),
        ("a_mode", C.c_int32), ("in_act", C.c_int32), ("in_slope", C.c_float),
        ("in_scale", C.c_void_p), ("in_shift", C.c_void_p),
        ("xyz", C.c_void_p), ("xyz_bstride", C.c_int64),
        ("nbr_idx", C.c_void_p), ("nbr_d2", C.c_void_p), ("nbr_k", C.c_int32),
        ("B", C.c_int32), ("n", C.c_int32), ("N", C.c_int32), ("K", C.c_int32),
        ("dY", C.c_void_p), ("lddy", C.c_int64), ("dy_bstride", C.c_int64),
        ("dW", C.c_void_p), ("w_ks", C.c_int64), ("w_ns", C.c_int64),
        ("dbias", C.c_void_p),
        ("slab", C.c_void_p), ("slab_floats", C.c_int64),
        ("defer_reduce", C.c_int32), ("rows_bf16", C.c_int32),
        ("a2_split", C.c_int32), ("a2_act", C.c_int32), ("A2", C.c_void_p), ("lda2", C.c_int64), ("a2_bstride", C.c_int64),
        ("a2_idx", C.c_void_p), ("a2_scale", C.c_void_p), ("a2_shift", C.c_void_p), ("a2_slope", C.c_float),
    ]


class WgradReduceItem(C.Structure):
    _fields_ = [
        ("slab", C.c_void_p), ("dW", C.c_void_p), ("dbias", C.c_void_p),
        ("w_ks", C.c_int64), ("w_ns", C.c_int64),
        ("nsplit", C.c_int32), ("N", C.c_int32), ("K", C.c_int32), ("reserved", C.c_int32),
    ]


class CloudJob(C.Structure):
    _fields_ = [
        ("xyz", C.c_void_p), ("features", C.c_void_p), ("labels", C.c_void_p), ("n_points", C.c_int64),
        ("xyz_f64", C.c_int32), ("normalization", C.c_int32), ("augment", C.c_int32), ("normal_col", C.c_int32),
        ("jitter_variance", C.c_double), ("jitter_limit", C.c_double), ("scale", C.c_double),
        ("R", C.c_double * 9), ("shift", C.c_double * 3),
    ]


class HeadDesc(C.Structure):
    _fields_ = [
        ("X", C.c_void_p), ("scale", C.c_void_p), ("shift", C.c_void_p), ("act", C.c_int32), ("slope", C.c_float),
        ("mean", C.c_void_p), ("invstd", C.c_void_p), ("W", C.c_void_p), ("bias", C.c_void_p),
        ("perm", C.c_void_p), ("labels", C.c_void_p), ("B", C.c_int32), ("N", C.c_int32), ("C", C.c_int32),
        ("loss_kind", C.c_int32), ("alpha", C.c_float), ("gamma", C.c_float), ("neglect_background", C.c_int32),
        ("drop_p", C.c_float), ("drop_key", C.c_void_p), ("drop_seed", C.c_uint64), ("drop_first_row", C.c_int64),
        ("work", C.c_void_p), ("G", C.c_void_p), ("bn_bwd_stats", C.c_void_p), ("slab", C.c_void_p),
        ("slab_floats", C.c_int64), ("grad_scale", C.c_float), ("reserved", C.c_int32), ("drop_mask", C.c_void_p), ("perm_bstride", C.c_int64),
        ("class_weight", C.c_void_p), ("masked", C.c_int32),
# ... 126 lines not shown
    "rl_wgrad_slab_floats": (_l, [_l, _i, _i]),
    "rl_set_wide_gemm": (_i, [C.c_char_p]),
    "rl_get_wide_gemm": (C.c_char_p, []),
    "rl_set_wgemm_staging": (_i, [C.c_char_p]),
    "rl_set_wgemm_tile": (_i, [C.c_char_p]),
    "rl_set_gemm_ksplit": (_i, [_i]),
    "rl_set_sgemm_grid_div": (_i, [_i]),
    "rl_wgrad": (_i, [C.POINTER(WgradDesc), _vp]),
    "rl_wgrad_plan": (_i, [C.POINTER(WgradDesc), C.POINTER(C.c_int32), C.POINTER(C.c_int32), C.POINTER(C.c_char_p)]),
    "rl_wgrad_nsplit": (_i, [_l, _i, _i]),
    "rl_wgrad_batchable": (_i, [C.POINTER(WgradDesc)]),
    "rl_wgrad_batch": (_i, [C.POINTER(WgradDesc), _i, _vp]),
    "rl_wgrad_reduce_batch": (_i, [C.POINTER(WgradReduceItem), _i, _vp]),
    "rl_bn_finalize": (_i, [_vp, _i, _l, _i, _vp, _vp, _vp, _vp, _vp, _f, _f, _i, _vp, _vp, _vp, _vp, _vp, _i, _vp, _vp]),
    "rl_bn_finalize_batch": (_i, [C.POINTER(BnFinalizeItem), _i, _vp]),
    "rl_bn_bwd_finalize_batch": (_i, [C.POINTER(BnBwdFinalizeItem), _i, _vp]),
    "rl_head_supported": (_i, [_i, _i]),
    "rl_head_grid": (_i, [_l]),
    "rl_head_fwd": (_i, [C.POINTER(HeadDesc), _vp, _vp]),
    "rl_head_bwd": (_i, [C.POINTER(HeadDesc), _vp]),
    "rl_bn_bwd_finalize_pair": (_i, [_vp, _vp, _i, _l, _i, _vp, _vp, _vp, _vp, _vp, _vp, _vp]),
    "rl_bn_reduce_slots": (_i, [_vp, _i, _i, _vp, _vp]),
    "rl_bn_bwd_slots": (_i, [_l]),
    "rl_bn_bwd_reduce": (_i, [C.POINTER(BnBwdDesc), _vp]),
    "rl_bn_bwd_finalize": (_i, [_vp, _i, _l, _i, _vp, _vp, _vp, _vp]),
    "rl_bn_bwd_apply": (_i, [C.POINTER(BnBwdDesc), _vp]),
    "rl_bn_bwd_fused_supported": (_i, [_l, _i, _l]),
    "rl_bn_bwd_fused": (_i, [C.POINTER(BnBwdDesc), _l, _vp, _vp, _vp, _vp]),
    "rl_resid_bn_bwd_supported": (_i, [_l, _i]),
    "rl_resid_bn_bwd_reduce": (_i, [C.POINTER(ResidBnBwdDesc), _vp]),
    "rl_resid_bn_bwd_apply": (_i, [C.POINTER(ResidBnBwdDesc), _vp]),
    "rl_resid_bn_bwd_fused_supported": (_i, [_l, _i]),
    "rl_resid_bn_bwd_fused": (_i, [C.POINTER(ResidBnBwdDesc), _vp, _vp, _vp, _vp, _vp]),
    "rl_copy_rows": (_i, [C.POINTER(RowsDesc), _vp]),
    "rl_copy_rows_pair": (_i, [C.POINTER(RowsDesc), C.POINTER(RowsDesc), _vp]),
    "rl_scatter_add_rows": (_i, [C.POINTER(RowsDesc), _vp]),
    "rl_csr_workspace_bytes": (_l, [C.POINTER(CsrTask), _i, _i]),
    "rl_csr_build": (_i, [C.POINTER(CsrTask), _i, _i, _vp, _l, _vp]),
    "rl_segment_sum_rows": (_i, [C.POINTER(SegsumDesc), _vp]),
    "rl_pool_supported": (_i, [_i, _i]),
    "rl_pool_slab_floats": (_l, [_l, _i]),
    "rl_pool_bwd_slots": (_i, [_l, _i]),
    "rl_pool_bwd_grid": (_i, [_l, _i, _i]),
    "rl_pool_fwd_slots": (_i, [_l, _i]),
    "rl_pool_fwd": (_i, [C.POINTER(PoolDesc), _vp]),
    "rl_rpe_stats_slots": (_i, [_l]),
    "rl_rpe_stats": (_i, [C.POINTER(PoolDesc), _vp, _vp]),
    "rl_rpe_bn_reduce": (_i, [C.POINTER(PoolDesc), _vp, _vp, _vp]),
    "rl_rpe_wgrad_slab_floats": (_l, [_l, _i, _i]),
    "rl_rpe_wgrad": (_i, [C.POINTER(PoolDesc), _vp, _vp, _vp, _l, _vp, _vp]),
    "rl_pool_bwd": (_i, [C.POINTER(PoolDesc), _vp]),
    "rl_set_pool128_x": (_i, [C.c_char_p]),
    "rl_get_pool128_x": (C.c_char_p, []),
    "rl_attpool_fwd": (_i, [_vp, _vp, _l, _i, _i, _vp, _vp]),
    "rl_attpool_bwd": (_i, [_vp, _vp, _vp, _vp, _l, _i, _i, _vp, _vp, _vp]),
    "rl_add_act_fwd": (_i, [_vp, _vp, _vp, _vp, _vp, _vp, _l, _i, _f, _vp, _vp]),
    "rl_add_act_bwd": (_i, [_vp, _vp, _l, _i, _f, _vp]),
    "rl_rpe_build": (_i, [_vp, _l, _vp, _vp, _i, _i, _i, _vp, _vp]),
    "rl_rpe_build_dist": (_i, [_vp, _l, _vp, _vp, _i, _i, _i, _vp, _vp]),
    "rl_batch_assemble": (_i, [_vp, _i, _i, _i, _vp, _vp, _vp, _vp, _vp, _vp]),
    "rl_batch_assemble_scratch_doubles": (_l, [_i, _i]),
    "rl_batch_assemble_flag_u32": (_l, [_i, _i, _i]),
    "rl_batch_draw": (_i, [_vp, _i, _i, C.c_uint64, _vp, _vp, _vp]),
    "rl_scale_mask": (_i, [_vp, _vp, _f, _l, _vp]),
    "rl_dropout_tick": (_i, [_vp, _vp, _vp]),
    "rl_dropout_fwd": (_i, [_vp, _vp, _vp, _i, _f, _vp, _l, _l, _i, _vp, C.c_uint64, _f, _vp]),
    "rl_dropout_bwd": (_i, [_vp, _l, _l, _i, _vp, C.c_uint64, _f, _vp]),
    "rl_upsample_cf": (_i, [_vp, _vp, _vp, _i, _i, _i, _i, _i, _i, _vp, _vp]),
    "rl_logits_unpermute": (_i, [_vp, _vp, _i, _i, _i, _vp, _vp]),
    "rl_logits_permute_grad": (_i, [_vp, _vp, _i, _i, _i, _vp, _vp]),
    "rl_logits_unpermute_b": (_i, [_vp, _vp, C.c_int64, _i, _i, _i, _vp, _vp]),
    "rl_logits_permute_grad_b": (_i, [_vp, _vp, C.c_int64, _i, _i, _i, _vp, _vp]),
    "rl_band_sort_workspace_bytes": (C.c_int64, [_i, _i, _vp, _i]),
    "rl_band_sort": (_i, [_vp, C.c_int64, _vp, _i, _i, _vp, _i, _vp, _vp, C.c_int64, _vp]),
    "rl_loss_max_classes": (_i, []),
    "rl_loss_work_doubles": (_l, [_l, _i]),
    "rl_loss_forward": (_i, [_vp, _vp, _i, _i, _i, _i, _f, _f, _i, _vp, _vp, _vp]),
    "rl_loss_backward": (_i, [_vp, _vp, _i, _i, _i, _i, _f, _f, _i, _vp, _f, _vp, _vp]),
    "rl_loss_forward_masked": (_i, [_vp, _vp, _i, _i, _i, _i, _f, _f, _i, _vp, _i, _vp, _vp, _vp]),
    "rl_loss_backward_masked": (_i, [_vp, _vp, _i, _i, _i, _i, _f, _f, _i, _vp, _f, _vp, _i, _vp, _vp]),
    "rl_loss_partials": (_i, [_vp, _vp, _i, _i, _i, _i, _f, _vp, _vp]),
    "rl_loss_totals_offset": (_l, [_i]),
    "rl_loss_from_totals": (_i, [_l, _i, _i, _f, _f, _i, _vp, _vp, _vp]),
    "rl_loss_backward_global": (_i, [_vp, _vp, _i, _i, _i, _i, _f, _f, _i, _vp, _f, _l, _vp, _vp]),
    "rl_lovasz_workspace_bytes": (_l, [_i, _i, _i]),
    "rl_lovasz_coef_offset": (_l, [_i, _i, _i]),
    "rl_lovasz_forward": (_i, [_vp, _vp, _i, _i, _i, _i, _vp, _vp, _l, _vp, _vp]),
    "rl_lovasz_backward": (_i, [_vp, _vp, _i, _i, _i, _i, _vp, _vp, _l, _f, _vp, _vp]),
    "rl_softmax_cf": (_i, [_vp, _i, _i, _i, _vp, _vp]),
    "rl_adam_step": (_i, [_vp, _vp, _vp, _vp, _l, _vp, _f, _f, _f, _f, _vp, _vp]),
    "rl_scene_workspace_bytes": (_l, [_l, _i]),
    "rl_scene_crop": (_i, [_vp, _l, _i, _vp, _i, _vp, _l, _vp, _vp, _l, _vp]),
    "rl_scene_accumulate": (_i, [_vp, _i, _i, _vp, _f, _f, _vp, _vp, _l, _vp]),
    "rl_scene_min_count": (_i, [_vp, _l, _vp, _vp, _vp]),
    "rl_scene_crop_padded": (_i, [_vp, _l, _i, _vp, _i, _vp, _l, _vp, _vp, _l, _vp]),
    "rl_scene_accumulate_first": (_i, [_vp, _i, _i, _vp, _f, _f, _vp, _vp, _l, _l, _i, _vp]),
    "rl_scenes_workspace_bytes": (_l, [_i, _l, _i]),
    "rl_scenes_init": (_i, [_vp, _i, _l, _vp, _vp, _l, _vp]),
    "rl_scenes_crop": (_i, [_vp, _i, _i, _l, _vp, _i, _i, _vp, _vp, _vp, _vp, _l, _vp]),
    "rl_scenes_crop_padded": (_i, [_vp, _i, _i, _l, _vp, _i, _i, _vp, _vp, _vp, _vp, _l, _vp]),
    "rl_scenes_vote_crop": (_i, [_vp, _i, _i, _l, _vp, _vp, _vp, _i, _i, _i, _i, _vp, _l, _l, _vp, _vp, _vp, _vp, _vp, _l, _vp]),
    "rl_scenes_vote_accumulate": (_i, [_vp, _i, _i, _l, _l, _i, _vp, _vp, _f, _f, _vp, _l, _vp]),
    "rl_grid_workspace_bytes": (_l, [_l, _i]),
    "rl_grid_bounds": (_i, [_vp, _l, _i, _f, _vp, _vp, _l, _vp]),
    "rl_grid_sort": (_i, [_vp, _l, _i, _i, _vp, _l, _vp]),
    "rl_grid_heads": (_i, [_l, _i, _vp, _vp, _vp, _l, _vp]),
# ... 81 lines not shown
```

### 3d_recognizer_amd/randlanet/_ops.py

```python
import contextlib
import ctypes as C
import os
from dataclasses import dataclass
from typing import Optional, Tuple

import torch

from . import _hip as H

F32 = torch.float32
BF16 = torch.bfloat16

_STORAGE = os.environ.get("RL_STORAGE", "f32")


def set_storage(mode: str) -> None:
    global _STORAGE
    if mode not in ("f32", "bf16"):
        raise ValueError(f"storage must be 'f32' or 'bf16', got {mode!r}")
    if mode == "bf16" and get_wide_gemm() == "fp32":
        raise H.HipKernelError("bf16 storage needs the bf16x3 / bf16 arithmetic mode (RL_WIDE_GEMM)")
    _STORAGE = mode


# ... 203 lines not shown
def set_wgemm_staging(how: str) -> None:
    H.check(H.lib().rl_set_wgemm_staging(how.encode()), "rl_set_wgemm_staging")


def set_wgemm_tile(how: str) -> None:
    H.check(H.lib().rl_set_wgemm_tile(how.encode()), "rl_set_wgemm_tile")


def set_gemm_ksplit(enable: bool) -> None:
    H.check(H.lib().rl_set_gemm_ksplit(int(bool(enable))), "rl_set_gemm_ksplit")


def rpe_build(a: "Rpe", distances: bool = False) -> Lazy:
    _dev_check(a.xyz, a.idx, a.d2)
    assert a.idx.dtype == torch.int32 and a.idx.shape == (a.B, a.n, a.K) and a.d2.shape == a.idx.shape
    assert a.xyz.shape[0] == a.B and a.xyz.shape[1] >= a.n and a.xyz.shape[2] == 3
    out = torch.empty((a.rows, 12), dtype=F32, device=a.xyz.device)
    with _rec("rpe_build", (a.rows,), (48 + 8) * a.rows, 0):
        fn = H.lib().rl_rpe_build_dist if distances else H.lib().rl_rpe_build
        H.check(fn(a.xyz.data_ptr(), a.xyz.shape[1], a.idx.data_ptr(), a.d2.data_ptr(), a.B, a.n, a.K,
                   out.data_ptr(), _st()), "rl_rpe_build")
    return Lazy(out, a.B, a.n * a.K, a.n * a.K, 10)


@dataclass
class ConcatGather:
    u: Lazy
    g: Lazy
    idx: torch.Tensor

    @property
    def B(self) -> int:
        return self.u.B

    @property
    def n(self) -> int:
        return self.u.n

    @property
    def C(self) -> int:
        return self.u.C + self.g.C

    @property
    def rows(self) -> int:
        return self.u.rows


def set_pool128_x(mode: str) -> None:
    H.check(H.lib().rl_set_pool128_x(mode.encode()), "rl_set_pool128_x")


def get_pool128_x() -> str:
    return H.lib().rl_get_pool128_x().decode()


def _fill_a(d, a):
    if isinstance(a, ConcatGather):
        u, g, idx = a.u, a.g, a.idx
        _dev_check(g.raw, g.scale, g.shift, idx)
        assert idx.dtype == torch.int32 and idx.numel() == u.rows and u.bstride == u.n and g.B == u.B
        assert g.raw.dtype == F32 and g.raw.dim() == 2 and g.raw.shape[1] >= g.C
        assert g.raw.shape[0] >= (g.B - 1) * g.bstride + g.n, "second source rows out of range"
        M, _ = _fill_a(d, u)
        d.K = u.C + g.C
        d.a2_split, d.A2, d.lda2, d.a2_bstride, d.a2_idx = u.C, g.raw.data_ptr(), g.raw.shape[1], g.bstride, idx.data_ptr()
        if g.scale is not None:
            assert g.scale.numel() == g.C and g.shift.numel() == g.C
            d.a2_scale, d.a2_shift, d.a2_act, d.a2_slope = g.scale.data_ptr(), g.shift.data_ptr(), g.act, g.slope
        return M, u.C + g.C
    if isinstance(a, Rpe):
        _dev_check(a.xyz, a.idx, a.d2)
        assert a.idx.dtype == torch.int32 and a.idx.shape == (a.B, a.n, a.K) and a.d2.shape == a.idx.shape
        assert a.xyz.shape[0] == a.B and a.xyz.shape[1] >= a.n and a.xyz.shape[2] == 3
        d.a_mode = 1
        d.xyz, d.xyz_bstride = a.xyz.data_ptr(), a.xyz.shape[1]
        d.nbr_idx, d.nbr_d2, d.nbr_k = a.idx.data_ptr(), a.d2.data_ptr(), a.K
        d.B, d.n, d.K = a.B, a.n, 10
        return a.rows, 10
    _dev_check(a.raw, a.scale, a.shift)
    assert a.raw.dtype in (F32, BF16) and a.raw.dim() == 2 and a.raw.shape[1] >= a.C
    assert a.raw.shape[0] >= (a.B - 1) * a.bstride + a.n, "A operand rows out of range"
    d.a_mode = 0
    d.A, d.lda, d.a_bstride = a.raw.data_ptr(), a.raw.shape[1], a.bstride
    if a.scale is not None:
        assert a.scale.numel() == a.C and a.shift.numel() == a.C
        d.in_scale, d.in_shift, d.in_act, d.in_slope = a.scale.data_ptr(), a.shift.data_ptr(), a.act, a.slope
    d.B, d.n, d.K = a.B, a.n, a.C
    return a.rows, a.C


def weight_strides(W: torch.Tensor, transposed: bool, K: int, N: int) -> Tuple[int, int]:
    if transposed:
        assert W.shape[0] == K and W.shape[1] == N, (tuple(W.shape), K, N)
        return N, 1
    assert W.shape[0] == N and W.shape[1] == K, (tuple(W.shape), K, N)
    return 1, K




def split_weights(entries) -> dict:
    out_map = {}
    if get_wide_gemm() == "fp32" or not entries:
        return out_map
    entries = [e[:5] for e in entries if e[3] % 8 == 0 and (e[4] > 64 or e[3] > 64 or len(e) > 5)]
    if not entries:
        return out_map
    total = sum(2 * K * N + 8 for _, _, _, K, N in entries)
    buf = torch.empty(total, dtype=torch.bfloat16, device=entries[0][0].device)
    arr = (H.WsplitItem * len(entries))()
    off = 0
    for it, (W, ks, ns, K, N) in zip(arr, entries):
        _dev_check(W)
        assert W.dtype == F32 and W.numel() == K * N
        out = buf[off:off + 2 * K * N]
        it.W, it.w_ks, it.w_ns, it.K, it.N, it.out = W.data_ptr(), ks, ns, K, N, out.data_ptr()
        out_map[(W.data_ptr(), ks, ns, K, N)] = out
        off += (2 * K * N + 7) // 8 * 8
    with _rec("split_weights", (len(entries),), 6 * sum(K * N for _, _, _, K, N in entries), 0):
        H.check(H.lib().rl_split_weights(arr, len(entries), _st()), "rl_split_weights")
    return out_map


def gemm_stat_slots(M: int, N: int, K: int) -> int:
    return int(H.lib().rl_gemm_stat_slots(M, N, K))


def gemm(a, W: torch.Tensor, w_ks: int, w_ns: int, N: int, bias: Optional[torch.Tensor] = None, *,
         out: Optional[torch.Tensor] = None, out_bstride: Optional[int] = None,
         accumulate: bool = False, stats: Optional[torch.Tensor] = None,
         addend: Optional[torch.Tensor] = None, out2: Optional[torch.Tensor] = None,
         out2_index: Optional[torch.Tensor] = None, out2_bstride: int = 0, split_col: int = 0,
         wsplit: Optional[dict] = None, pivot: Optional[tuple] = None, bnb: Optional[Lazy] = None):
    d = H.GemmDesc()
    M, K = _fill_a(d, a)
    assert isinstance(a, Rpe) or a.raw.dtype == F32, "rl_gemm reads fp32 rows"
    rows_per_batch = a.n * a.K if isinstance(a, Rpe) else a.n
    _dev_check(W, bias, out, stats)
    assert W.dtype == F32 and W.numel() == K * N
    if out is None:
        out = torch.empty((M, N), dtype=F32, device=W.device)
        out_bstride = rows_per_batch
    else:
        assert out.dtype == F32 and out.dim() == 2 and out.shape[1] >= (split_col if out2 is not None else N)
        out_bstride = rows_per_batch if out_bstride is None else out_bstride
        assert out.shape[0] >= (d.B - 1) * out_bstride + rows_per_batch, "Y rows out of range"
    if bias is not None:
        assert bias.numel() == N
    if stats is not None:
        assert stats.dtype == torch.float64 and stats.numel() >= gemm_stat_slots(M, N, K) * 2 * N
    d.N, d.W, d.w_ks, d.w_ns, d.bias = N, W.data_ptr(), w_ks, w_ns, H.ptr(bias)
    planes = wsplit.get((W.data_ptr(), w_ks, w_ns, K, N)) if wsplit else None
    if planes is not None:
        d.W_split = planes.data_ptr()
    d.Y, d.ldy, d.y_bstride, d.accumulate = out.data_ptr(), out.shape[1], out_bstride, int(accumulate)
    d.stats = H.ptr(stats)
    if pivot is not None:
        assert stats is not None and pivot[0].numel() == N and (pivot[1] is None or pivot[1].numel() == N)
        _dev_check(*pivot)
        d.stats_pivot_mean, d.stats_pivot_bias = pivot[0].data_ptr(), H.ptr(pivot[1])
    if addend is not None or out2 is not None:
        _dev_check(addend, out2, out2_index)
        assert addend is None or (addend.dtype == F32 and addend.shape == (M, N))
        if out2 is not None:
            assert out2.dtype == F32 and 0 < split_col < N and out2.shape[1] == N - split_col
            if out2_index is None:
                assert out2.shape[0] >= M
            else:
                assert out2_index.dtype == torch.int32 and out2_index.numel() == M
                assert out2.shape[0] >= (d.B - 1) * out2_bstride + 1
        d.addend, d.out2, d.out2_index = H.ptr(addend), H.ptr(out2), H.ptr(out2_index)
        d.out2_bstride, d.split_col = out2_bstride, split_col
    bnb_pre = None
    if bnb is not None:
        if (stats is None and pivot is None and bnb.mean is not None and bnb.scale is not None and bnb.raw.dtype == F32
                and bnb.raw.shape[1] == out.shape[1] and bnb.bstride == out_bstride and bnb.C == N
                and 4 * M * N <= BNB_MAX_BYTES and H.lib().rl_gemm_streams(C.byref(d))):
            _dev_check(bnb.raw, bnb.scale, bnb.shift, bnb.mean, bnb.invstd)
            st_b = new_stats(W.device, N)
            d.stats = st_b.data_ptr()
            d.bnb_Y, d.bnb_scale, d.bnb_shift = bnb.raw.data_ptr(), bnb.scale.data_ptr(), bnb.shift.data_ptr()
            d.bnb_mean, d.bnb_invstd, d.bnb_act, d.bnb_slope = bnb.mean.data_ptr(), bnb.invstd.data_ptr(), bnb.act, bnb.slope
            bnb_pre = (st_b, gemm_stat_slots(M, N, K))
    kfloats = H.lib().rl_gemm_kslab_floats(M, N, K) if (N > 64 and not isinstance(a, Rpe) and out2 is None and addend is None) else 0
    if kfloats > 0:
        kslab = _slab(W.device, kfloats)
        d.kslab, d.kslab_floats = kslab.data_ptr(), kslab.numel()
    with _rec("gemm_rpe" if isinstance(a, Rpe) else "gemm", (M, K, N), 4 * (M * (K if not isinstance(a, Rpe) else 6) + M * N * (2 if accumulate else 1) + K * N), 2 * M * K * N):
        H.check(H.lib().rl_gemm(C.byref(d), _st()), "rl_gemm")
    return (out, bnb_pre) if bnb is not None else out


BNB_MAX_BYTES = 32 << 20


def gemm_pair(a, first: tuple, second: tuple, wsplit: Optional[dict]):
    if not wsplit or isinstance(a, Rpe) or a.raw.dtype != F32:
        return None
    descs, outs = [], []
    M = K = None
    for (W, w_ks, w_ns, N, stats, pivot) in (first, second):
        d = H.GemmDesc()
        M, K = _fill_a(d, a)
        planes = wsplit.get((W.data_ptr(), w_ks, w_ns, K, N))
        if planes is None:
            return None
        _dev_check(W, stats)
        out = torch.empty((M, N), dtype=F32, device=W.device)
        d.N, d.W, d.w_ks, d.w_ns, d.W_split = N, W.data_ptr(), w_ks, w_ns, planes.data_ptr()
        d.Y, d.ldy, d.y_bstride = out.data_ptr(), N, a.n
        if stats is not None:
            assert stats.dtype == torch.float64 and stats.numel() >= H.row_blocks(M, 128) * 2 * N
            d.stats = stats.data_ptr()
            if pivot is not None:
                _dev_check(*pivot)
                d.stats_pivot_mean, d.stats_pivot_bias = pivot[0].data_ptr(), H.ptr(pivot[1])
        descs.append(d)
        outs.append(out)
    if not H.lib().rl_gemm_pair_supported(C.byref(descs[0]), C.byref(descs[1])):
        return None
    N1, N2 = first[3], second[3]
    with _rec("gemm", (M, K, N1 + N2), 4 * (M * K + M * (N1 + N2) + K * (N1 + N2)), 2 * M * K * (N1 + N2)):
        H.check(H.lib().rl_gemm_pair(C.byref(descs[0]), C.byref(descs[1]), _st()), "rl_gemm_pair")
    return outs[0], outs[1]


_SLAB = {}


def _slab(device, floats: int) -> torch.Tensor:
    key = (device, torch.cuda.current_stream(device).cuda_stream)
    buf = _SLAB.get(key)
    if buf is None or buf.numel() < floats:
        buf = torch.empty(max(floats, 1 << 20), dtype=F32, device=device)
        _SLAB[key] = buf
    return buf


WGRAD_BATCH_BYTES = 3 << 30


def wgrad(a, dY: torch.Tensor, dy_bstride: int, N: int, dW: torch.Tensor, w_ks: int, w_ns: int,
          dbias: Optional[torch.Tensor] = None, pending: Optional[list] = None, batch: Optional[list] = None) -> None:
# ... 533 lines not shown
    pd = _pool_desc(u, g, idx, W, n, d, stage)
    _dev_check(dP, GU, dW)
    P = u.B * n
    assert dP.shape == (P, d) and GU.shape == (P * 16, d // 2) and dW.numel() == d * d
    rdt = row_dtype()
    virt = isinstance(u, VirtualRpe)
    assert GU.dtype == (rdt if virt else F32), "GU: the row storage type under a virtual rpe branch, fp32 for a real U tensor"
    pd.rows_bf16 = int(rdt == BF16)
    es = 2 if rdt == BF16 else 4
    DG = torch.empty((P * 16, d // 2), dtype=rdt, device=W.device)
    if bn_bwd_stats is not None:
        _dev_check(bn_bwd_stats)
        assert stage > 0 and bn_bwd_stats.dtype == torch.float64
        assert bn_bwd_stats.numel() >= H.lib().rl_pool_bwd_slots(P, d) * d
        pd.bn_bwd_stats = bn_bwd_stats.data_ptr()
    pd.dP, pd.GU, pd.gu_accumulate, pd.DG, pd.dW = dP.data_ptr(), GU.data_ptr(), int(gu_accumulate), DG.data_ptr(), dW.data_ptr()
    h = d // 2
    if virt:
        nbytes = P * (4 * (32 + d) + 16 * (16 + 4 * h) + 4 * d + es * 16 * h * (2 + int(gu_accumulate)))
    else:
        nbytes = (4 * (2 * P * 16 * h + P * 16 + 2 * P * d) + es * P * 16 * h + 4 * P * 16 * h * (1 + int(gu_accumulate)))
    if d == 128:
        dS = torch.empty((P * 16, d), dtype=rdt, device=W.device)
        xop = ConcatGather(u, g, idx) if (rdt == F32 and not virt and get_pool128_x() == "in_place") else None
        if xop is not None and not wgrad_supported(xop, dS, n * 16, d):
            xop = None
        if xop is None:
            X = torch.empty((P * 16, d), dtype=rdt, device=W.device)
            pd.X_out, xop = X.data_ptr(), plain(X, u.B, n * 16)
        else:
            pd.x_optional = 1
        pd.dS_out = dS.data_ptr()
        with _rec("pool_bwd", (P, 16, d), nbytes + (1 + int(pd.x_optional == 0)) * es * P * 16 * d, 4 * P * 16 * d * d):
            H.check(H.lib().rl_pool_bwd(C.byref(pd), _st()), "rl_pool_bwd")
        wgrad(xop, dS, n * 16, d, dW, 1, d, None, pending=pending, batch=batch)
        return DG
    floats = H.lib().rl_pool_slab_floats(P, d)
    if pending is not None:
        slab = torch.empty(floats, dtype=F32, device=W.device)
        pd.dW = None
    else:
        slab = _slab(W.device, floats)
    pd.slab, pd.slab_floats = slab.data_ptr(), slab.numel()
    with _rec("pool_bwd", (P, 16, d), nbytes, 6 * P * 16 * d * d):
        H.check(H.lib().rl_pool_bwd(C.byref(pd), _st()), "rl_pool_bwd")
    if pending is not None:
        it = H.WgradReduceItem()
        it.slab, it.dW, it.dbias, it.w_ks, it.w_ns = slab.data_ptr(), dW.data_ptr(), None, 1, d
        it.nsplit, it.N, it.K = H.lib().rl_pool_bwd_grid(P, d, int(virt)), d, d
        pending.append((it, slab, dW, None))
    return DG


def attpool_fwd(X: torch.Tensor, S: torch.Tensor, P: int, K: int) -> torch.Tensor:
    _dev_check(X, S)
    Cc = X.shape[1]
    assert X.shape == S.shape == (P * K, Cc)
    out = torch.empty((P, Cc), dtype=F32, device=X.device)
    with _rec("attpool_fwd", (P, K, Cc), 4 * (2 * P * K * Cc + P * Cc), 0):
        H.check(H.lib().rl_attpool_fwd(X.data_ptr(), S.data_ptr(), P, K, Cc, out.data_ptr(), _st()), "rl_attpool_fwd")
    return out


def attpool_bwd(X, S, Pout, dP, P: int, K: int):
    _dev_check(X, S, Pout, dP)
    Cc = X.shape[1]
    assert X.shape == S.shape == (P * K, Cc) and Pout.shape == dP.shape == (P, Cc)
    dS = torch.empty_like(S)
    dXa = torch.empty_like(X)
    with _rec("attpool_bwd", (P, K, Cc), 4 * (4 * P * K * Cc + 2 * P * Cc), 0):
        H.check(H.lib().rl_attpool_bwd(X.data_ptr(), S.data_ptr(), Pout.data_ptr(), dP.data_ptr(), P, K, Cc,
                                       dS.data_ptr(), dXa.data_ptr(), _st()), "rl_attpool_bwd")
    return dS, dXa


def add_act_fwd(y1: Lazy, y2: Lazy, slope: float) -> torch.Tensor:
    assert y1.rows == y2.rows and y1.C == y2.C and y1.bstride == y1.n and y2.bstride == y2.n
    out = torch.empty((y1.rows, y1.C), dtype=F32, device=y1.raw.device)
    with _rec("add_act", (y1.rows, y1.C), 12 * y1.rows * y1.C, 0):
        H.check(H.lib().rl_add_act_fwd(y1.raw.data_ptr(), y1.scale.data_ptr(), y1.shift.data_ptr(), y2.raw.data_ptr(),
                                       y2.scale.data_ptr(), y2.shift.data_ptr(), y1.rows, y1.C, slope, out.data_ptr(),
                                       _st()), "rl_add_act_fwd")
    return out


def add_act_bwd(G: torch.Tensor, O: torch.Tensor, slope: float) -> None:
    assert G.shape == O.shape and G.is_contiguous() and O.is_contiguous()
    with _rec("add_act", (G.shape[0], G.shape[1]), 12 * G.numel(), 0):
        H.check(H.lib().rl_add_act_bwd(G.data_ptr(), O.data_ptr(), G.shape[0], G.shape[1], slope, _st()), "rl_add_act_bwd")


def scale_mask(x: torch.Tensor, mask: torch.Tensor, scale: float) -> None:
    _dev_check(x, mask)
    assert mask.dtype == torch.uint8 and mask.numel() == x.numel() and x.dtype == F32
    H.check(H.lib().rl_scale_mask(x.data_ptr(), mask.data_ptr(), scale, x.numel(), _st()), "rl_scale_mask")


def dropout_tick(counter: torch.Tensor) -> torch.Tensor:
    _dev_check(counter)
    assert counter.dtype == torch.int64 and counter.numel() == 1
    key = torch.empty(1, dtype=torch.int64, device=counter.device)
    H.check(H.lib().rl_dropout_tick(counter.data_ptr(), key.data_ptr(), _st()), "rl_dropout_tick")
    return key


def dropout_fwd(x: Lazy, key: torch.Tensor, seed: int, p: float, first_row: int = 0) -> torch.Tensor:
    _dev_check(x.raw, x.scale, x.shift, key)
    assert x.bstride == x.n and x.raw.shape == (x.rows, x.C) and x.C % 4 == 0
    out = torch.empty_like(x.raw)
    with _rec("dropout", (x.rows, x.C), 8 * x.rows * x.C, 0):
        H.check(H.lib().rl_dropout_fwd(x.raw.data_ptr(), H.ptr(x.scale), H.ptr(x.shift), x.act, x.slope, out.data_ptr(),
                                       x.rows, first_row, x.C, key.data_ptr(), seed & 0xFFFFFFFFFFFFFFFF, p, _st()), "rl_dropout_fwd")
    return out


def dropout_bwd(G: torch.Tensor, key: torch.Tensor, seed: int, p: float, first_row: int = 0) -> None:
    _dev_check(G, key)
    assert G.dim() == 2 and G.shape[1] % 4 == 0
    with _rec("dropout", (G.shape[0], G.shape[1]), 8 * G.numel(), 0):
        H.check(H.lib().rl_dropout_bwd(G.data_ptr(), G.shape[0], first_row, G.shape[1], key.data_ptr(), seed & 0xFFFFFFFFFFFFFFFF, p,
                                       _st()), "rl_dropout_bwd")

# ... 704 lines not shown
```

### include/rl_randlanet.h

```cpp
#ifndef RL_RANDLANET_H
#define RL_RANDLANET_H

#include <stdint.h>

#ifdef __cplusplus
extern "C" {
#endif

#define RL_VERSION 110

#define RL_OK 0
#define RL_ERR_ARGS (-1)
#define RL_ERR_FEW_SUPPORT (-2)
#define RL_ERR_LAUNCH (-3)
#define RL_ERR_UNSUPPORTED (-4)

#define RL_MAX_SLOTS 1024
#define RL_KNN_MAX_K 64
#define RL_MAX_CLASSES 256

const char* rl_last_error(void);
const char* rl_last_kernel(void);
int rl_version(void);
int64_t rl_launch_count(void);
// ... 15 lines not shown

typedef struct rl_knn_task {
    const float* support;
    int64_t support_bstride;
    const float* query;
    int64_t query_bstride;
    int32_t Ns, Nq, k;
    int32_t* idx_out;
    float* d2_out;
} rl_knn_task;

int64_t rl_knn_multi_workspace_bytes(const rl_knn_task* tasks, int ntasks, int B);
int rl_knn_multi(const rl_knn_task* tasks, int ntasks, int B, void* workspace, int64_t workspace_bytes,
                 void* stream);

typedef struct rl_gemm_desc {
    const float* A;
    int64_t lda, a_bstride;
    int32_t a_mode;
    int32_t in_act;
    float in_slope;
    const float* in_scale;
    const float* in_shift;
    const float* xyz;
    int64_t xyz_bstride;
    const int32_t* nbr_idx;
    const float* nbr_d2;
    int32_t nbr_k;
    int32_t B, n, N, K;
    const float* W;
    int64_t w_ks, w_ns;
    const float* bias;
    float* Y;
    int64_t ldy, y_bstride;
    int32_t accumulate;
    double* stats;
    float* kslab;
    int64_t kslab_floats;
    const float* addend;
    float* out2;
    const int32_t* out2_index;
    int64_t out2_bstride;
    int32_t split_col;
    const void* W_split;
    const float* stats_pivot_mean;
    const float* stats_pivot_bias;
    const float* bnb_Y;
    const float* bnb_scale;
    const float* bnb_shift;
    const float* bnb_mean;
    const float* bnb_invstd;
    int32_t bnb_act;
    float bnb_slope;
} rl_gemm_desc;

int rl_gemm_streams(const rl_gemm_desc* d);
int rl_gemm_pair_supported(const rl_gemm_desc* a, const rl_gemm_desc* b);
int rl_gemm_pair(const rl_gemm_desc* a, const rl_gemm_desc* b, void* stream);

typedef struct rl_wsplit_item {
    const float* W;
    int64_t w_ks, w_ns;
    int32_t K, N;
    void* out;
} rl_wsplit_item;

int rl_split_weights(const rl_wsplit_item* items, int count, void* stream);

int64_t rl_gemm_kslab_floats(int64_t M, int N, int K);
int64_t rl_gemm_stat_slots(int64_t M, int N, int K);

int rl_set_wide_gemm(const char* mode);
const char* rl_get_wide_gemm(void);
int rl_set_wgemm_staging(const char* how);
int rl_set_wgemm_tile(const char* how);
int rl_set_gemm_ksplit(int enable);
int rl_set_sgemm_grid_div(int div);
int rl_gemm(const rl_gemm_desc* d, void* stream);

typedef struct rl_wgrad_desc {
    const float* A;
    int64_t lda, a_bstride;
    int32_t a_mode;
    int32_t in_act;
    float in_slope;
    const float* in_scale;
    const float* in_shift;
    const float* xyz;
    int64_t xyz_bstride;
    const int32_t* nbr_idx;
    const float* nbr_d2;
    int32_t nbr_k;
    int32_t B, n, N, K;
    const float* dY;
    int64_t lddy, dy_bstride;
    float* dW;
    int64_t w_ks, w_ns;
    float* dbias;
    float* slab;
    int64_t slab_floats;
    int32_t defer_reduce;
    int32_t rows_bf16;
    int32_t a2_split;
    int32_t a2_act;
    const float* A2;
    int64_t lda2, a2_bstride;
    const int32_t* a2_idx;
    const float* a2_scale;
    const float* a2_shift;
// ... 99 lines not shown

typedef struct rl_rows_desc {
    const float* src;
    int64_t lds, src_bstride;
    float* dst;
    int64_t ldd;
    int64_t rows, rows_per_batch;
    int32_t C;
    const int32_t* index32;
    const int64_t* index64;
    int32_t index_shared;
    int32_t accumulate;
    int32_t act;
    float slope;
    const float* scale;
    const float* shift;
} rl_rows_desc;

int rl_copy_rows(const rl_rows_desc* d, void* stream);
int rl_copy_rows_pair(const rl_rows_desc* d0, const rl_rows_desc* d1, void* stream);

int rl_scatter_add_rows(const rl_rows_desc* d, void* stream);

typedef struct rl_csr_task {
    const int32_t* idx;
    int32_t n_src, k, n_dst;
    int32_t* offsets;
    int32_t* entries;
} rl_csr_task;

int64_t rl_csr_workspace_bytes(const rl_csr_task* tasks, int ntasks, int B);
int rl_csr_build(const rl_csr_task* tasks, int ntasks, int B, void* workspace, int64_t workspace_bytes,
                 void* stream);

typedef struct rl_segsum_desc {
    const float* src;
    int64_t lds, src_bstride;
    float* dst;
    int64_t ldd, dst_bstride;
    const int32_t* offsets;
    const int32_t* entries;
    int64_t entries_per_cloud;
    int32_t B, n_dst, C;
    int32_t accumulate;
    int32_t src_bf16;
} rl_segsum_desc;

int rl_segment_sum_rows(const rl_segsum_desc* d, void* stream);

int rl_attpool_fwd(const float* X, const float* S, int64_t P, int K, int C, float* Pout,
                   void* stream);
int rl_attpool_bwd(const float* X, const float* S, const float* Pout, const float* dP, int64_t P,
                   int K, int C, float* dS, float* dXa, void* stream);

typedef struct rl_pool_desc {
    const float* U;
    const float* u_scale;
    const float* u_shift;
    int32_t u_act;
    float u_slope;
    const float* G;
    int64_t g_bstride;
    const float* g_scale;
    const float* g_shift;
    int32_t g_act;
    float g_slope;
    const int32_t* idx;
    const float* W;
    int64_t points;
    int32_t n, d, nbr_k;
    float* Pout;
    const float* dP;
    float* GU;
    int32_t gu_accumulate;
    float* DG;
    float* dW;
    float* slab;
    int64_t slab_floats;
    float* X_out;
    float* dS_out;
    int32_t u_source;
    const float* xyz;
    int64_t xyz_bstride;
    const float* nbr_d2;
    const float* W1;
    const float* b1;
    const float* scale1;
    const float* shift1;
    const float* W2;
    const float* b2;
    const float* scale2;
    const float* shift2;
    const float* mean1;
    const float* invstd1;
    const float* mean2;
    const float* invstd2;
    int32_t xyz_width;
    double* bn_bwd_stats;
    double* bn_fwd_stats2;
    int32_t rows_bf16;
    const float* pivot_mean1;
    const float* pivot_mean2;
    int32_t x_optional;
} rl_pool_desc;

int rl_pool_supported(int d, int nbr_k);
// ... 234 lines not shown
```

Measured before the change: 1293.

## Fuse concat-gather A operand into wide GEMM and attentive pooling kernels

```diff
diff --git a/3d_recognizer_amd/csrc/gemm.hip b/3d_recognizer_amd/csrc/gemm.hip
--- a/3d_recognizer_amd/csrc/gemm.hip
+++ b/3d_recognizer_amd/csrc/gemm.hip
@@ -93,6 +93,15 @@
         As[r * stride + c] = v;
     }
 }
+
+struct ConcatSrc {
+    const float* A2;
+    const int32_t* idx;
+    const float* sc2; const float* sh2;
+    long a2_bstride;
+    int lda2, split, act2;
+    float slope2;
+};
 
 struct GemmParams {
     AOperand a;
@@ -256,15 +265,6 @@
 constexpr int WG_T = 64;
 constexpr int WG_S = 80;
 
-struct ConcatSrc {
-    const float* A2;
-    const int32_t* idx;
-    const float* sc2; const float* sh2;
-    long a2_bstride;
-    int lda2, split, act2;
-    float slope2;
-};
-
 struct WgradParams {
     AOperand a;
     ConcatSrc cat;
@@ -1509,6 +1509,9 @@
 }
 
 typedef __attribute__((address_space(3))) unsigned char rl_lds_byte;
+typedef int rl_i32x8 __attribute__((ext_vector_type(8)));
+typedef __attribute__((address_space(4))) unsigned char rl_const_byte;
+typedef __attribute__((address_space(4), aligned(4))) rl_i32x8 rl_const_i32x8;
 __device__ __forceinline__ unsigned lds_address(const void* q) {
     return (unsigned)(uintptr_t)(const rl_lds_byte*)q;
 }
@@ -1550,8 +1553,8 @@
 #endif
 constexpr int W2_KMAX = 1024;
 constexpr int W2_THREADS = 768;
-template <int TERMS, bool STATS, int AS, int WS, int BM = 128, int BN = 128>
-__global__ __launch_bounds__(W2_THREADS) void wgemm2_kernel(const GemmParams pk) {
+template <int TERMS, bool STATS, int AS, int WS, int BM, int BN, bool CAT>
+__device__ __forceinline__ void wgemm2_body(const GemmParams& pk, const ConcatSrc& cs) {
     static_assert(AS >= 3 && AS <= 6 && WS >= 2 && WS <= 6, "ring depths vs the wait table");
     static_assert((BM == 128 || BM == 64) && (BN == 128 || BN == 64), "tile shapes");
     constexpr int RB = BM / 16;
@@ -1583,12 +1586,22 @@
     const int K = p.a.K, N = p.N;
     const long M = p.a.M;
     const long ntiles = (M + BM - 1) / BM;
-    const bool lazy = p.a.lazy.scale != nullptr;
+    constexpr bool cat = CAT;
+    const bool lazy = cat || p.a.lazy.scale != nullptr;
     float* lsc = reinterpret_cast<float*>(lds + OFF_SC);
     float* lsh = lsc + W2_KMAX;
     double* red = reinterpret_cast<double*>(lds + OFF_RED);
     const unsigned lds0 = lds_address(lds);
-    if (lazy) {
+    if (cat) {
+        for (int k = tid; k < K; k += W2_THREADS) {
+            const bool two = k >= cs.split;
+            const int c = two ? k - cs.split : k;
+            const float* scp = two ? cs.sc2 : p.a.lazy.scale;
+            const float* shp = two ? cs.sh2 : p.a.lazy.shift;
+            lsc[k] = scp ? scp[c] : 1.f;
+            lsh[k] = scp ? shp[c] : 0.f;
+        }
+    } else if (lazy) {
         for (int k = tid; k < K; k += W2_THREADS) {
             lsc[k] = p.a.lazy.scale[k];
             lsh[k] = p.a.lazy.shift[k];
@@ -1645,14 +1658,38 @@
         constexpr int AI = BM / 16;
         const int lw = wave - 8;
         const float* asrc[AI];
+        const float* asrc2[AI];
+        int nidx[AI];
+        auto group_row = [&](int j, int i) {
+            long Rg = ((long)bx + (long)j * p.gx) * BM + (lw * AI + i) * 8;
+            return Rg < M ? Rg : M - 8;
+        };
+        auto fetch_idx = [&](int j) {
+            const int sub = lane >> 3;
+            rl_i32x8 g[AI];
+#pragma unroll
+            for (int i = 0; i < AI; ++i) g[i] = *(const rl_const_i32x8*)((const rl_const_byte*)cs.idx + group_row(j, i) * 4);
+#pragma unroll
+            for (int i = 0; i < AI; ++i) {
+                int gi = g[i][0];
+                gi = sub == 1 ? g[i][1] : gi; gi = sub == 2 ? g[i][2] : gi; gi = sub == 3 ? g[i][3] : gi; gi = sub == 4 ? g[i][4] : gi;
+                gi = sub == 5 ? g[i][5] : gi; gi = sub == 6 ? g[i][6] : gi; gi = sub == 7 ? g[i][7] : gi;
+                nidx[i] = gi;
+            }
+        };
         auto tile_sources = [&](int j) {
             const long row0 = ((long)bx + (long)j * p.gx) * BM;
 #pragma unroll
             for (int i = 0; i < AI; ++i) {
                 const int r = (lw * AI + i) * 8 + (lane >> 3);
+                const int seg = ((lane & 7) ^ ((r >> 1) & 7)) << 2;
                 long R = row0 + r;
                 R = R < M ? R : M - 1;
-                asrc[i] = p.a.A + a_row_offset(p.a, R) + (((lane & 7) ^ ((r >> 1) & 7)) << 2) + k_begin;
+                const long Rg = group_row(j, i);
+                if (cat) R = Rg + (lane >> 3);
+                asrc[i] = p.a.A + a_row_offset(p.a, R) + seg + k_begin;
+                const unsigned b = cat ? (unsigned)Rg / (unsigned)p.a.n : 0u;
+                asrc2[i] = cat ? cs.A2 + ((long)b * cs.a2_bstride + nidx[i]) * cs.lda2 + seg - cs.split : asrc[i];
             }
         };
         int iq = 0, ic = 0;
@@ -1660,11 +1697,19 @@
             if (ic == 0) tile_sources(iq / nch);
             const int k = ic * PG_BK;
             const unsigned l = __builtin_amdgcn_readfirstlane(lds0 + (iq % AS) * A_STAGE + lw * AI * 1024);
-            glds16x4(asrc[0] + k, asrc[1] + k, asrc[2] + k, asrc[3] + k, l, l + 1024, l + 2048, l + 3072);
-            if constexpr (AI == 8) glds16x4(asrc[4] + k, asrc[5] + k, asrc[6] + k, asrc[7] + k, l + 4096, l + 5120, l + 6144, l + 7168);
+            const bool two = cat && k >= cs.split;
+            const float* s[AI];
+#pragma unroll
+            for (int i = 0; i < AI; ++i) s[i] = (two ? asrc2[i] : asrc[i]) + k;
+            glds16x4(s[0], s[1], s[2], s[3], l, l + 1024, l + 2048, l + 3072);
+            if constexpr (AI == 8) glds16x4(s[4], s[5], s[6], s[7], l + 4096, l + 5120, l + 6144, l + 7168);
+            if (cat && ic == 0 && iq / nch + 1 < my_tiles) fetch_idx(iq / nch + 1);
             ++iq;
             ic = ic + 1 == nch ? 0 : ic + 1;
         };
+#pragma unroll
+        for (int i = 0; i < AI; ++i) nidx[i] = 0;
+        if (cat && T > 0) fetch_idx(0);
         while (iq < AS - 1 && iq < T) issue_a();
         for (int q = 0; q < T; ++q) {
             wait_vm_chunks<AI>(min(AS - 2, T - 1 - q));
@@ -1675,6 +1720,13 @@
         const int lr = lane & 15, lq = lane >> 4;
         const bool relu = p.a.lazy.act == RL_ACT_RELU;
         const float nslope = p.a.lazy.act == RL_ACT_NONE ? 1.f : p.a.lazy.slope;
+        float e_one = 1.f, e_two = 1.f;
+        if (cat) {
+            RlLazy t2 = p.a.lazy;
+            t2.scale = cs.sc2; t2.shift = cs.sh2; t2.act = cs.act2; t2.slope = cs.slope2;
+            e_one = rl_eff_slope(p.a.lazy);
+            e_two = rl_eff_slope(t2);
+        }
         const int rb = wave % RB, cg = wave / RB;
         const int cg0 = cg * NT * 16;
         const int frow = rb * 16 + lr;
@@ -1696,7 +1748,16 @@
             const unsigned char* Wb = lds + OFF_W + (q % WS) * W_STAGE;
             float4 v0 = *reinterpret_cast<const float4*>(Ab + a_frag0);
             float4 v1 = *reinterpret_cast<const float4*>(Ab + a_frag1);
-            if (lazy) {
+            if (cat) {
+                const int kk = c * PG_BK + lq * 8;
+                const float e = c * PG_BK >= cs.split ? e_two : e_one;
+                const f32x4 x0 = rl_fold_act4((f32x4){v0.x, v0.y, v0.z, v0.w}, *reinterpret_cast<const f32x4*>(lsc + kk),
+                                              *reinterpret_cast<const f32x4*>(lsh + kk), e);
+                const f32x4 x1 = rl_fold_act4((f32x4){v1.x, v1.y, v1.z, v1.w}, *reinterpret_cast<const f32x4*>(lsc + kk + 4),
+                                              *reinterpret_cast<const f32x4*>(lsh + kk + 4), e);
+                v0 = make_float4(x0[0], x0[1], x0[2], x0[3]);
+                v1 = make_float4(x1[0], x1[1], x1[2], x1[3]);
+            } else if (lazy) {
                 const int kk = k_begin + c * PG_BK + lq * 8;
                 const float4 sc0 = *reinterpret_cast<const float4*>(lsc + kk), sc1 = *reinterpret_cast<const float4*>(lsc + kk + 4);
                 const float4 sh0 = *reinterpret_cast<const float4*>(lsh + kk), sh1 = *reinterpret_cast<const float4*>(lsh + kk + 4);
@@ -1820,6 +1881,15 @@
             }
         }
     }
+}
+
+template <int TERMS, bool STATS, int AS, int WS, int BM = 128, int BN = 128>
+__global__ __launch_bounds__(W2_THREADS) void wgemm2_kernel(const GemmParams pk) {
+    wgemm2_body<TERMS, STATS, AS, WS, BM, BN, false>(pk, ConcatSrc{});
+}
+template <int TERMS, bool STATS, int AS, int WS, int BM = 128, int BN = 128>
+__global__ __launch_bounds__(W2_THREADS) void wgemm2_cat_kernel(const GemmParams pk, const ConcatSrc cs) {
+    wgemm2_body<TERMS, STATS, AS, WS, BM, BN, true>(pk, cs);
 }
 
 constexpr int WS_MAX = 64;
@@ -2546,6 +2616,7 @@
 
 
 typedef void (*GemmFn)(const GemmParams);
+typedef void (*GemmCatFn)(const GemmParams, const ConcatSrc);
 typedef void (*WgradFn)(const WgradParams);
 enum GemmKernel { GK_NONE, GK_SGEMM, GK_PGEMM, GK_WGEMM, GK_WGEMM2, GK_GEMM };
 
@@ -2555,11 +2626,14 @@
     bool pgemm, wgemm, wgemm2;
     bool split, stats, bnb;
     int64_t kslab_floats;
+    int cat_split;
+    int rows_per_cloud;
 };
 
 struct GemmPlan {
     GemmKernel kernel;
     GemmFn fn;
+    GemmCatFn catfn;
     int threads; dim3 grid;
     WidePlan wide;
     int gx, ny, ksplit, kchunk;
@@ -2582,6 +2656,15 @@
     return w.bm == 128 ? wgemm2_kernel<TERMS, STATS, W2_AS, W2_WS, 128, 128>
          : w.bn == 128 ? wgemm2_kernel<TERMS, STATS, W2_AS, W2_WS, 64, 128> : wgemm2_kernel<TERMS, STATS, W2_AS, W2_WS, 64, 64>;
 }
+template <int TERMS, bool STATS>
+GemmCatFn wide_cat_inst(WidePlan w) {
+    return w.bm == 128 ? wgemm2_cat_kernel<TERMS, STATS, W2_AS, W2_WS, 128, 128>
+         : w.bn == 128 ? wgemm2_cat_kernel<TERMS, STATS, W2_AS, W2_WS, 64, 128> : wgemm2_cat_kernel<TERMS, STATS, W2_AS, W2_WS, 64, 64>;
+}
+inline GemmCatFn wide_cat_fn(bool stats, WidePlan w) {
+    if (wide_gemm_terms() == 1) return stats ? wide_cat_inst<1, true>(w) : wide_cat_inst<1, false>(w);
+    return stats ? wide_cat_inst<3, true>(w) : wide_cat_inst<3, false>(w);
+}
 inline GemmFn wide_fn(bool stats, bool dma, WidePlan w) {
     if (wide_gemm_terms() == 1) return stats ? wide_inst<1, true>(dma, w) : wide_inst<1, false>(dma, w);
     return stats ? wide_inst<3, true>(dma, w) : wide_inst<3, false>(dma, w);
@@ -2608,7 +2691,29 @@
     pl.name = dma ? (splitk ? "wgemm2_kernel+splitk" : "wgemm2_kernel") : (splitk ? "wgemm_kernel+splitk" : "wgemm_kernel");
 }
 
+GemmPlan plan_gemm(const GemmFacts& f);
+GemmPlan plan_gemm_concat(GemmFacts f) {
+    const int split = f.cat_split, n = f.rows_per_cloud;
+    f.cat_split = 0;
+    f.streamable = true;
+    GemmPlan pl = plan_gemm(f);
+    if (pl.kernel == GK_NONE) return pl;
+    if (!(pl.kernel == GK_WGEMM2 && pl.ksplit == 1 && pl.wide.ksplit == 1 && !pl.reduce && f.K == 2 * split && split % PG_BK == 0 &&
+          f.K <= W2_KMAX && n % 16 == 0 && f.M % 16 == 0)) {
+        pl.kernel = GK_NONE;
+        pl.fn = nullptr;
+        pl.refusal = "rl_gemm: a concat-gather A operand (a2_split) needs the LDS-DMA wide kernel in one pass (bf16x3 / bf16 arithmetic, "
+                     "pre-split weight, dma staging, no K split), fp32 rows, K == 2 * a2_split <= 1024, a2_split % 32 == 0 and rows per "
+                     "cloud a multiple of 16";
+        return pl;
+    }
+    pl.catfn = wide_cat_fn(f.stats, pl.wide);
+    pl.name = "wgemm2_kernel<cat>";
+    return pl;
+}
+
 GemmPlan plan_gemm(const GemmFacts& f) {
+    if (f.cat_split != 0) return plan_gemm_concat(f);
     const int N = f.N, K = f.K, nt = N <= 16 ? 1 : N <= 32 ? 2 : N <= 64 ? 4 : 8;
     GemmPlan pl{};
     pl.threads = 256; pl.ksplit = 1;
@@ -2669,12 +2774,13 @@
 
 inline GemmFacts aligned_facts(long M, int N, int K, bool dma) {
     return GemmFacts{M, N, K, true, true, wide_gemm_terms() != 0 && K % 8 == 0,
-                     dma && wgemm_staging() == 1 && K % PG_BK == 0 && K <= W2_KMAX, false, true, false, 0};
-}
-
-int launch_gemm(const GemmPlan& pl, hipStream_t st, GemmParams p, const char* who) {
+                     dma && wgemm_staging() == 1 && K % PG_BK == 0 && K <= W2_KMAX, false, true, false, 0, 0, 0};
+}
+
+int launch_gemm(const GemmPlan& pl, hipStream_t st, GemmParams p, const char* who, const ConcatSrc* cat = nullptr) {
     p.gx = pl.gx; p.ny = pl.ny; p.ksplit = pl.ksplit; p.kchunk = pl.kchunk;
-    hipLaunchKernelGGL(pl.fn, pl.grid, dim3(pl.threads), 0, st, p);
+    if (pl.catfn && cat) hipLaunchKernelGGL(pl.catfn, pl.grid, dim3(pl.threads), 0, st, p, *cat);
+    else hipLaunchKernelGGL(pl.fn, pl.grid, dim3(pl.threads), 0, st, p);
     rl_note_kernel(pl.name);
     RL_LAUNCH_CHECK(who);
     if (!pl.reduce) return RL_OK;
@@ -2781,13 +2887,28 @@
     return t == 0 ? "fp32" : t == 1 ? "bf16" : "bf16x3";
 }
 
-extern "C" int rl_gemm(const rl_gemm_desc* d, void* stream) {
+static int gemm_fill(const rl_gemm_desc* d, GemmParams* pp, GemmPlan* plan, ConcatSrc* cs) {
     RL_REQUIRE(d != nullptr, RL_ERR_ARGS, "rl_gemm: null descriptor");
-    GemmParams p{};
+    GemmParams& p = *pp;
+    p = GemmParams{};
+    *cs = ConcatSrc{};
+    const int cat = d->a2_split;
+    RL_REQUIRE(cat == 0 || (cat > 0 && cat < d->K && d->a_mode == 0), RL_ERR_ARGS,
+               "rl_gemm: a2_split must lie inside (0, K), on a tensor operand");
     int rc = fill_a(&p.a, "rl_gemm", d->A, d->lda, d->a_bstride, d->a_mode, d->in_act, d->in_slope,
                     d->in_scale, d->in_shift, d->xyz, d->xyz_bstride, d->nbr_idx, d->nbr_d2, d->nbr_k,
-                    d->B, d->n, d->K);
+                    d->B, d->n, cat ? cat : d->K);
     if (rc) return rc;
+    p.a.K = d->K;
+    if (cat) {
+        RL_REQUIRE(d->A2 && d->a2_idx && d->a2_bstride > 0 && (d->a2_scale == nullptr) == (d->a2_shift == nullptr), RL_ERR_ARGS,
+                   "rl_gemm: incomplete second source (A2, a2_idx, a2_bstride; a2_scale / a2_shift come together)");
+        RL_REQUIRE((((uintptr_t)d->A2) & 15) == 0 && d->lda2 % 4 == 0 && d->lda2 >= d->K - cat && d->lda2 < (1l << 31) &&
+                   (((uintptr_t)d->a2_idx) & 3) == 0, RL_ERR_ARGS,
+                   "rl_gemm: A2 must be 16-byte aligned with lda2 a multiple of 4 and >= K - a2_split");
+        cs->A2 = d->A2; cs->idx = d->a2_idx; cs->sc2 = d->a2_scale; cs->sh2 = d->a2_shift;
+        cs->a2_bstride = d->a2_bstride; cs->lda2 = (int)d->lda2; cs->split = cat; cs->act2 = d->a2_act; cs->slope2 = d->a2_slope;
+    }
     RL_REQUIRE(d->N > 0 && d->W && d->Y && d->ldy > 0, RL_ERR_ARGS, "rl_gemm: bad W/Y");
     p.N = d->N; p.W = d->W; p.w_ks = d->w_ks; p.w_ns = d->w_ns; p.bias = d->bias;
     p.Y = d->Y; p.ldy = d->ldy; p.y_bstride = d->y_bstride;
@@ -2813,7 +2934,7 @@
     }
     p.stat_slots = (int)rl_gemm_stat_slots(p.a.M, d->N, d->K);
     const GemmPlan pl = plan_gemm(GemmFacts{p.a.M, d->N, d->K, p.a.a_mode == 0 && p.a.vec4p, pgemm_ok(p), wgemm_ok(p), wgemm2_usable(p),
-                                            split, d->stats != nullptr, d->bnb_Y != nullptr, d->kslab ? d->kslab_floats : 0});
+                                            split, d->stats != nullptr, d->bnb_Y != nullptr, d->kslab ? d->kslab_floats : 0, cat, d->n});
     RL_REQUIRE(pl.kernel != GK_NONE, RL_ERR_UNSUPPORTED, "%s", pl.refusal);
     if (!split && d->bnb_Y) {
         RL_REQUIRE(d->stats && d->bnb_scale && d->bnb_shift && d->bnb_mean && d->bnb_invstd && !d->stats_pivot_mean, RL_ERR_ARGS,
@@ -2823,13 +2944,29 @@
         p.piv_mean = p.piv_bias = nullptr;
     }
     p.kslab = pl.reduce ? d->kslab : nullptr;
-    return launch_gemm(pl, (hipStream_t)stream, p, "rl_gemm");
+    *plan = pl;
+    return RL_OK;
+}
+
+extern "C" int rl_gemm(const rl_gemm_desc* d, void* stream) {
+    GemmParams p;
+    GemmPlan pl;
+    ConcatSrc cs;
+    const int rc = gemm_fill(d, &p, &pl, &cs);
+    return rc ? rc : launch_gemm(pl, (hipStream_t)stream, p, "rl_gemm", cs.split > 0 ? &cs : nullptr);
+}
+
+extern "C" int rl_gemm_concat_supported(const rl_gemm_desc* d) {
+    GemmParams p;
+    GemmPlan pl;
+    ConcatSrc cs;
+    return gemm_fill(d, &p, &pl, &cs);
 }
 
 extern "C" int rl_gemm_streams(const rl_gemm_desc* d) {
     if (!d) return 0;
     const bool vec4p = (d->lda % 4 == 0) && ((d->K + 3) / 4 * 4 <= d->lda) && (((uintptr_t)d->A & 15) == 0);
-    const GemmFacts f{(long)d->B * d->n, d->N, d->K, d->a_mode == 0 && vec4p, false, false, false, d->addend || d->out2, false, false, 0};
+    const GemmFacts f{(long)d->B * d->n, d->N, d->K, d->a_mode == 0 && vec4p, false, false, false, d->addend || d->out2, false, false, 0, 0, 0};
     return (plan_gemm(f).kernel == GK_SGEMM && d->N <= 64) ? 1 : 0;
 }
 
diff --git a/3d_recognizer_amd/csrc/rl_common.h b/3d_recognizer_amd/csrc/rl_common.h
--- a/3d_recognizer_amd/csrc/rl_common.h
+++ b/3d_recognizer_amd/csrc/rl_common.h
@@ -109,6 +109,10 @@
     if (t.scale == nullptr || t.act == RL_ACT_NONE) return 1.f;
     return t.act == RL_ACT_RELU ? 0.f : t.slope;
 }
+inline float rl_eff_slope_host(const RlLazy& t) {
+    if (t.scale == nullptr || t.act == RL_ACT_NONE) return 1.f;
+    return t.act == RL_ACT_RELU ? 0.f : t.slope;
+}
 __device__ __forceinline__ rl_f32x4 rl_fold_act4(const rl_f32x4 raw, const rl_f32x4 scale, const rl_f32x4 shift, const float e) {
     const rl_f32x4 z = raw * scale + shift;
     const rl_f32x4 ev = {e, e, e, e};
diff --git a/3d_recognizer_amd/csrc/rows.hip b/3d_recognizer_amd/csrc/rows.hip
--- a/3d_recognizer_amd/csrc/rows.hip
+++ b/3d_recognizer_amd/csrc/rows.hip
@@ -1,3 +1,5 @@
+#include <string.h>
+
 #include "rl_common.h"
 
 namespace {
@@ -131,9 +133,46 @@
     return (int)(g < 4096 ? g : 4096);
 }
 
-template <typename I>
+struct AttCat {
+    const float* U; const float* G; const int32_t* idx;
+    const float* u_scale; const float* u_shift; const float* g_scale; const float* g_shift;
+    long ldu, ldg, g_bstride;
+    int h, n;
+    float e_u, e_g;
+};
+typedef int rl_i32x16 __attribute__((ext_vector_type(16)));
+typedef __attribute__((address_space(4), aligned(4))) rl_i32x16 rl_const_i32x16;
+typedef __attribute__((address_space(4))) unsigned char rl_const_byte;
+__device__ __forceinline__ void attcat_x16(const AttCat& q, long pt, int c, float (&xv)[16]) {
+    const int ptu = __builtin_amdgcn_readfirstlane((int)pt);
+    const bool two = __builtin_amdgcn_readfirstlane(c) >= q.h;
+    const float* scp = two ? q.g_scale : q.u_scale;
+    const float* shp = two ? q.g_shift : q.u_shift;
+    const int ch = two ? c - q.h : c;
+    if (two) {
+        const rl_i32x16 id = *(const rl_const_i32x16*)((const rl_const_byte*)q.idx + (long)ptu * 64);
+        const int b = (int)((unsigned)ptu / (unsigned)q.n);
+        const float* g = q.G + (long)b * q.g_bstride * q.ldg + ch;
+#pragma unroll
+        for (int k = 0; k < 16; ++k) xv[k] = g[(long)id[k] * q.ldg];
+    } else {
+        const float* u = q.U + (long)ptu * 16 * q.ldu + ch;
+#pragma unroll
+        for (int k = 0; k < 16; ++k) xv[k] = u[(long)k * q.ldu];
+    }
+    if (scp) {
+        const float sc = scp[ch], sh = shp[ch], es = two ? q.e_g : q.e_u;
+#pragma unroll
+        for (int k = 0; k < 16; ++k) {
+            const float z = xv[k] * sc + sh;
+            xv[k] = __builtin_elementwise_max(z, z * es);
+        }
+    }
+}
+
+template <typename I, bool CAT = false>
 __global__ __launch_bounds__(256) void attpool_fwd16_kernel(const float* __restrict__ X, const float* __restrict__ S,
-                                                            long P, int C, float* __restrict__ Pout) {
+                                                            long P, int C, float* __restrict__ Pout, const AttCat q) {
     const long total = P * C;
     for (long e = (long)blockIdx.x * 256 + threadIdx.x; e < total; e += (long)gridDim.x * 256) {
         const long pt = (long)((I)e / (I)C);
@@ -143,8 +182,11 @@
         float sv[16], xv[16];
 #pragma unroll
         for (int k = 0; k < 16; ++k) sv[k] = s[(long)k * C];
-#pragma unroll
-        for (int k = 0; k < 16; ++k) xv[k] = x[(long)k * C];
+        if constexpr (CAT) attcat_x16(q, pt, c, xv);
+        else {
+#pragma unroll
+            for (int k = 0; k < 16; ++k) xv[k] = x[(long)k * C];
+        }
         float m = sv[0];
 #pragma unroll
         for (int k = 1; k < 16; ++k) m = fmaxf(m, sv[k]);
@@ -158,10 +200,11 @@
         Pout[e] = num / den;
     }
 }
-template <typename I>
+template <typename I, bool CAT = false>
 __global__ __launch_bounds__(256) void attpool_bwd16_kernel(const float* __restrict__ X, const float* __restrict__ S,
                                                             const float* __restrict__ Pout, const float* __restrict__ dP,
-                                                            long P, int C, float* __restrict__ dS, float* __restrict__ dXa) {
+                                                            long P, int C, float* __restrict__ dS, float* __restrict__ dXa,
+                                                            const AttCat q) {
     const long total = P * C;
     for (long e = (long)blockIdx.x * 256 + threadIdx.x; e < total; e += (long)gridDim.x * 256) {
         const long pt = (long)((I)e / (I)C);
@@ -170,8 +213,11 @@
         float sv[16], xv[16];
 #pragma unroll
         for (int k = 0; k < 16; ++k) sv[k] = S[base + (long)k * C];
-#pragma unroll
-        for (int k = 0; k < 16; ++k) xv[k] = X[base + (long)k * C];
+        if constexpr (CAT) attcat_x16(q, pt, c, xv);
+        else {
+#pragma unroll
+            for (int k = 0; k < 16; ++k) xv[k] = X[base + (long)k * C];
+        }
         const float g = dP[e], po = Pout[e];
         float m = sv[0];
 #pragma unroll
@@ -469,7 +515,7 @@
     RL_REQUIRE(X && S && Pout && P >= 0 && K > 0 && C > 0, RL_ERR_ARGS, "rl_attpool_fwd: bad arguments");
     if (P == 0) return RL_OK;
     if (fits32(P * C)) {
-        if (K == 16) hipLaunchKernelGGL(attpool_fwd16_kernel<uint32_t>, dim3(grid_for(P * C)), dim3(256), 0, (hipStream_t)stream, X, S, (long)P, C, Pout);
+        if (K == 16) hipLaunchKernelGGL(attpool_fwd16_kernel<uint32_t>, dim3(grid_for(P * C)), dim3(256), 0, (hipStream_t)stream, X, S, (long)P, C, Pout, AttCat{});
         else hipLaunchKernelGGL(attpool_fwd_kernel<uint32_t>, dim3(grid_for(P * C)), dim3(256), 0, (hipStream_t)stream, X, S, (long)P, K, C, Pout);
     } else {
         hipLaunchKernelGGL(attpool_fwd_kernel<int64_t>, dim3(grid_for(P * C)), dim3(256), 0, (hipStream_t)stream, X, S, (long)P, K, C, Pout);
@@ -485,7 +531,7 @@
     if (P == 0) return RL_OK;
     if (fits32(P * C) && K == 16)
         hipLaunchKernelGGL(attpool_bwd16_kernel<uint32_t>, dim3(grid_for(P * C)), dim3(256), 0, (hipStream_t)stream, X, S, Pout, dP,
-                           (long)P, C, dS, dXa);
+                           (long)P, C, dS, dXa, AttCat{});
     else if (fits32(P * C))
         hipLaunchKernelGGL(attpool_bwd_kernel<uint32_t>, dim3(grid_for(P * C)), dim3(256), 0, (hipStream_t)stream, X, S, Pout, dP,
                            (long)P, K, C, dS, dXa);
@@ -496,6 +542,60 @@
     RL_LAUNCH_CHECK("rl_attpool_bwd");
     return RL_OK;
 }
+
+static int attcat_fill(const rl_attpool_src* x, int64_t P, int K, int C, AttCat* q, const char* who) {
+    RL_REQUIRE(x && x->U && x->G && x->idx && x->n > 0 && x->h > 0 && x->g_bstride > 0, RL_ERR_ARGS, "%s: incomplete sources", who);
+    RL_REQUIRE((x->u_scale == nullptr) == (x->u_shift == nullptr) && (x->g_scale == nullptr) == (x->g_shift == nullptr), RL_ERR_ARGS,
+               "%s: scale / shift come together", who);
+    RL_REQUIRE(x->ldu >= x->h && x->ldg >= x->h && (((uintptr_t)x->idx) & 3) == 0, RL_ERR_ARGS, "%s: bad leading dimensions", who);
+    RL_REQUIRE(K == 16 && C == 2 * x->h && x->h % 64 == 0 && fits32(P * C) && P * 16 < (1l << 31), RL_ERR_UNSUPPORTED,
+               "%s: the in-place X needs K == 16, C == 2 * h, h %% 64 == 0 and fewer than 2^32 elements", who);
+    RlLazy lu{x->u_scale, x->u_shift, x->u_act, x->u_slope}, lg{x->g_scale, x->g_shift, x->g_act, x->g_slope};
+    *q = AttCat{x->U, x->G, x->idx, x->u_scale, x->u_shift, x->g_scale, x->g_shift, (long)x->ldu, (long)x->ldg, (long)x->g_bstride,
+                x->h, x->n, rl_eff_slope_host(lu), rl_eff_slope_host(lg)};
+    return RL_OK;
+}
+
+extern "C" int rl_attpool_cat_supported(const rl_attpool_src* x, int64_t P, int K, int C) {
+    AttCat q;
+    return attcat_fill(x, P, K, C, &q, "rl_attpool_cat_supported");
+}
+
+extern "C" int rl_attpool_fwd_cat(const rl_attpool_src* x, const float* S, int64_t P, int K, int C, float* Pout, void* stream) {
+    RL_REQUIRE(S && Pout && P >= 0 && C > 0, RL_ERR_ARGS, "rl_attpool_fwd_cat: bad arguments");
+    AttCat q;
+    const int rc = attcat_fill(x, P, K, C, &q, "rl_attpool_fwd_cat");
+    if (rc) return rc;
+    if (P == 0) return RL_OK;
+    hipLaunchKernelGGL((attpool_fwd16_kernel<uint32_t, true>), dim3(grid_for(P * C)), dim3(256), 0, (hipStream_t)stream,
+                       (const float*)nullptr, S, (long)P, C, Pout, q);
+    rl_note_kernel("attpool_fwd_kernel");
+    RL_LAUNCH_CHECK("rl_attpool_fwd_cat");
+    return RL_OK;
+}
+
+extern "C" int rl_attpool_bwd_cat(const rl_attpool_src* x, const float* S, const float* Pout, const float* dP, int64_t P, int K,
+                                  int C, float* dS, float* dXa, void* stream) {
+    RL_REQUIRE(S && Pout && dP && dS && dXa && P >= 0 && C > 0, RL_ERR_ARGS, "rl_attpool_bwd_cat: bad arguments");
+    AttCat q;
+    const int rc = attcat_fill(x, P, K, C, &q, "rl_attpool_bwd_cat");
+    if (rc) return rc;
+    if (P == 0) return RL_OK;
+    hipLaunchKernelGGL((attpool_bwd16_kernel<uint32_t, true>), dim3(grid_for(P * C)), dim3(256), 0, (hipStream_t)stream,
+                       (const float*)nullptr, S, Pout, dP, (long)P, C, dS, dXa, q);
+    rl_note_kernel("attpool_bwd_kernel");
+    RL_LAUNCH_CHECK("rl_attpool_bwd_cat");
+    return RL_OK;
+}
+
+static int g_pool256_x_in_place = 1;
+extern "C" int rl_set_pool256_x(const char* mode) {
+    const bool in_place = mode && !strcmp(mode, "in_place"), stored = mode && !strcmp(mode, "stored");
+    RL_REQUIRE(in_place || stored, RL_ERR_ARGS, "rl_set_pool256_x: mode must be \"in_place\" or \"stored\"");
+    g_pool256_x_in_place = in_place ? 1 : 0;
+    return RL_OK;
+}
+extern "C" const char* rl_get_pool256_x(void) { return g_pool256_x_in_place ? "in_place" : "stored"; }
 
 extern "C" int rl_add_act_fwd(const float* Y1, const float* s1, const float* b1, const float* Y2, const float* s2,
                               const float* b2, int64_t rows, int C, float slope, float* O, void* stream) {
diff --git a/3d_recognizer_amd/randlanet/_engine.py b/3d_recognizer_amd/randlanet/_engine.py
--- a/3d_recognizer_amd/randlanet/_engine.py
+++ b/3d_recognizer_amd/randlanet/_engine.py
@@ -11,6 +11,7 @@
 BN_MOMENTUM = 0.99
 BN_PIVOT = True
 BAND_SORT_MIN_POINTS = 4096
+POOL_X_IN_PLACE_MIN_ROWS = 2048
 
 
 @dataclass(slots=True, eq=False)
@@ -39,7 +40,7 @@
     u: Lazy
     g: Lazy
     csr: object
-    X: torch.Tensor
+    X: object
     S: torch.Tensor
     pooled: Lazy
     n: int
@@ -304,14 +305,30 @@
             pooled = ops.plain(res, B, n)
             ctx.record(PoolFusedRec(name, u, g, csr, idx, pooled, n, d, stage))
             return self._mlp(ctx, pooled, f"{name}.mlp", n_out, H.ACT_RELU)
-        X = torch.empty((rows, d), dtype=torch.float32, device=u.raw.device)
-        ops.copy_rows_pair(((u.raw, (0, h), n * K, X, (0, h), rows, n * K), dict(lazy=u)),
-                           ((g.raw, (0, h), g.bstride, X, (h, h), rows, n * K), dict(index=idx, lazy=g)))
-        S = ops.gemm(ops.plain(X, B, n * K), Ws, 1, d, d, None, wsplit=ctx.wsplit)
+        X = self._pool_x_in_place(ctx, u, g, idx, Ws, n, d)
+        if X is None:
+            X = torch.empty((rows, d), dtype=torch.float32, device=u.raw.device)
+            ops.copy_rows_pair(((u.raw, (0, h), n * K, X, (0, h), rows, n * K), dict(lazy=u)),
+                               ((g.raw, (0, h), g.bstride, X, (h, h), rows, n * K), dict(index=idx, lazy=g)))
+            S = ops.gemm(ops.plain(X, B, n * K), Ws, 1, d, d, None, wsplit=ctx.wsplit)
+        else:
+            S = ops.gemm(X, Ws, 1, d, d, None, wsplit=ctx.wsplit)
         Pt = ops.attpool_fwd(X, S, B * n, K)
         pooled = ops.plain(Pt, B, n)
         ctx.record(PoolRec(name, u, g, csr, X, S, pooled, n, d))
         return self._mlp(ctx, pooled, f"{name}.mlp", n_out, H.ACT_RELU)
+
+    def _pool_x_in_place(self, ctx, u, g: Lazy, idx: torch.Tensor, Ws: torch.Tensor, n: int, d: int):
+        K = self.K
+        if (ops.get_pool256_x() != "in_place" or not isinstance(u, Lazy) or u.rows <= POOL_X_IN_PLACE_MIN_ROWS
+                or u.raw.dtype != torch.float32 or g.raw.dtype != torch.float32 or ops.row_dtype() != torch.float32 or u.bstride != u.n):
+            return None
+        x = ops.ConcatGather(u, g, idx)
+        if not ops.attpool_concat_supported(x, u.B * n, K) or not ops.gemm_concat_supported(x, Ws, 1, d, d, ctx.wsplit):
+            return None
+        if ctx.training and not ops.wgrad_supported(x, Ws, n * K, d):
+            return None
+        return x
 
     def _virtual_bn(self, ctx: Context, vr, stage: int, bn_name: str, stats=None, nslots: int = 1) -> Lazy:
         if ctx.training and stats is None:
@@ -679,8 +696,8 @@
         GP = st.arrived(pooled).buf
         dS, dX = ops.attpool_bwd(X, S, pooled.raw, GP, B * n, K)
         Ws = self.P[f"{name}.score_fn.0.weight"]
-        ops.wgrad(ops.plain(X, B, n * K), dS, n * K, d, grads[f"{name}.score_fn.0.weight"], 1, d, None, pending=st.pending,
-                  batch=st.wbatch)
+        ops.wgrad(X if isinstance(X, ops.ConcatGather) else ops.plain(X, B, n * K), dS, n * K, d,
+                  grads[f"{name}.score_fn.0.weight"], 1, d, None, pending=st.pending, batch=st.wbatch)
         gu = st.slot(u)
         gg = st.slot(g)
         if d <= 64:
diff --git a/3d_recognizer_amd/randlanet/_hip.py b/3d_recognizer_amd/randlanet/_hip.py
--- a/3d_recognizer_amd/randlanet/_hip.py
+++ b/3d_recognizer_amd/randlanet/_hip.py
@@ -41,6 +41,18 @@
         ("stats_pivot_mean", C.c_void_p), ("stats_pivot_bias", C.c_void_p),
         ("bnb_Y", C.c_void_p), ("bnb_scale", C.c_void_p), ("bnb_shift", C.c_void_p), ("bnb_mean", C.c_void_p),
         ("bnb_invstd", C.c_void_p), ("bnb_act", C.c_int32), ("bnb_slope", C.c_float),
+        ("a2_split", C.c_int32), ("a2_act", C.c_int32), ("A2", C.c_void_p), ("lda2", C.c_int64), ("a2_bstride", C.c_int64),
+        ("a2_idx", C.c_void_p), ("a2_scale", C.c_void_p), ("a2_shift", C.c_void_p), ("a2_slope", C.c_float),
+    ]
+
+
+class AttpoolSrc(C.Structure):
+    _fields_ = [
+        ("U", C.c_void_p), ("ldu", C.c_int64), ("u_scale", C.c_void_p), ("u_shift", C.c_void_p), ("u_act", C.c_int32),
+        ("u_slope", C.c_float),
+        ("G", C.c_void_p), ("ldg", C.c_int64), ("g_bstride", C.c_int64), ("g_scale", C.c_void_p), ("g_shift", C.c_void_p),
+        ("g_act", C.c_int32), ("g_slope", C.c_float),
+        ("idx", C.c_void_p), ("n", C.c_int32), ("h", C.c_int32),
     ]
 
 
@@ -273,6 +285,12 @@
     "rl_pool_bwd": (_i, [C.POINTER(PoolDesc), _vp]),
     "rl_set_pool128_x": (_i, [C.c_char_p]),
     "rl_get_pool128_x": (C.c_char_p, []),
+    "rl_set_pool256_x": (_i, [C.c_char_p]),
+    "rl_get_pool256_x": (C.c_char_p, []),
+    "rl_gemm_concat_supported": (_i, [C.POINTER(GemmDesc)]),
+    "rl_attpool_cat_supported": (_i, [C.POINTER(AttpoolSrc), _l, _i, _i]),
+    "rl_attpool_fwd_cat": (_i, [C.POINTER(AttpoolSrc), _vp, _l, _i, _i, _vp, _vp]),
+    "rl_attpool_bwd_cat": (_i, [C.POINTER(AttpoolSrc), _vp, _vp, _vp, _l, _i, _i, _vp, _vp, _vp]),
     "rl_attpool_fwd": (_i, [_vp, _vp, _l, _i, _i, _vp, _vp]),
     "rl_attpool_bwd": (_i, [_vp, _vp, _vp, _vp, _l, _i, _i, _vp, _vp, _vp]),
     "rl_add_act_fwd": (_i, [_vp, _vp, _vp, _vp, _vp, _vp, _l, _i, _f, _vp, _vp]),
diff --git a/3d_recognizer_amd/randlanet/_ops.py b/3d_recognizer_amd/randlanet/_ops.py
--- a/3d_recognizer_amd/randlanet/_ops.py
+++ b/3d_recognizer_amd/randlanet/_ops.py
@@ -279,6 +279,14 @@
 
 def get_pool128_x() -> str:
     return H.lib().rl_get_pool128_x().decode()
+
+
+def set_pool256_x(mode: str) -> None:
+    H.check(H.lib().rl_set_pool256_x(mode.encode()), "rl_set_pool256_x")
+
+
+def get_pool256_x() -> str:
+    return H.lib().rl_get_pool256_x().decode()
 
 
 def _fill_a(d, a):
@@ -361,7 +369,8 @@
          wsplit: Optional[dict] = None, pivot: Optional[tuple] = None, bnb: Optional[Lazy] = None):
     d = H.GemmDesc()
     M, K = _fill_a(d, a)
-    assert isinstance(a, Rpe) or a.raw.dtype == F32, "rl_gemm reads fp32 rows"
+    cat = isinstance(a, ConcatGather)
+    assert isinstance(a, Rpe) or (a.u.raw if cat else a.raw).dtype == F32, "rl_gemm reads fp32 rows"
     rows_per_batch = a.n * a.K if isinstance(a, Rpe) else a.n
     _dev_check(W, bias, out, stats)
     assert W.dtype == F32 and W.numel() == K * N
@@ -409,13 +418,32 @@
             d.bnb_Y, d.bnb_scale, d.bnb_shift = bnb.raw.data_ptr(), bnb.scale.data_ptr(), bnb.shift.data_ptr()
             d.bnb_mean, d.bnb_invstd, d.bnb_act, d.bnb_slope = bnb.mean.data_ptr(), bnb.invstd.data_ptr(), bnb.act, bnb.slope
             bnb_pre = (st_b, gemm_stat_slots(M, N, K))
-    kfloats = H.lib().rl_gemm_kslab_floats(M, N, K) if (N > 64 and not isinstance(a, Rpe) and out2 is None and addend is None) else 0
+    kfloats = H.lib().rl_gemm_kslab_floats(M, N, K) if (N > 64 and not isinstance(a, Rpe) and not cat and out2 is None and addend is None) else 0
     if kfloats > 0:
         kslab = _slab(W.device, kfloats)
         d.kslab, d.kslab_floats = kslab.data_ptr(), kslab.numel()
-    with _rec("gemm_rpe" if isinstance(a, Rpe) else "gemm", (M, K, N), 4 * (M * (K if not isinstance(a, Rpe) else 6) + M * N * (2 if accumulate else 1) + K * N), 2 * M * K * N):
+    nbytes = 4 * (M * (K if not isinstance(a, Rpe) else 6) + M * N * (2 if accumulate else 1) + K * N)
+    if cat:
+        nbytes = 4 * (M * a.u.C + a.g.rows * a.g.C + M) + 4 * (M * N * (2 if accumulate else 1) + K * N)
+    with _rec("gemm_rpe" if isinstance(a, Rpe) else "gemm", (M, K, N), nbytes, 2 * M * K * N):
         H.check(H.lib().rl_gemm(C.byref(d), _st()), "rl_gemm")
     return (out, bnb_pre) if bnb is not None else out
+
+
+def gemm_concat_supported(a: ConcatGather, W: torch.Tensor, w_ks: int, w_ns: int, N: int, wsplit: Optional[dict]) -> bool:
+    if a.u.raw.dtype != F32 or a.g.raw.dtype != F32:
+        return False
+    d = H.GemmDesc()
+    M, K = _fill_a(d, a)
+    d.N, d.W, d.w_ks, d.w_ns = N, W.data_ptr(), w_ks, w_ns
+    planes = wsplit.get((W.data_ptr(), w_ks, w_ns, K, N)) if wsplit else None
+    if planes is not None:
+        d.W_split = planes.data_ptr()
+    d.Y, d.ldy, d.y_bstride = W.data_ptr(), N, a.n
+    rc = H.lib().rl_gemm_concat_supported(C.byref(d))
+    if rc not in (0, H.ERR_UNSUPPORTED):
+        H.check(rc, "rl_gemm_concat_supported")
+    return rc == 0
 
 
 BNB_MAX_BYTES = 32 << 20
@@ -1055,22 +1083,65 @@
     return DG
 
 
-def attpool_fwd(X: torch.Tensor, S: torch.Tensor, P: int, K: int) -> torch.Tensor:
+def _attpool_src(x: ConcatGather) -> H.AttpoolSrc:
+    u, g, idx = x.u, x.g, x.idx
+    _dev_check(u.raw, u.scale, u.shift, g.raw, g.scale, g.shift, idx)
+    assert idx.dtype == torch.int32 and idx.numel() == u.rows and u.bstride == u.n and g.B == u.B and u.C == g.C
+    assert u.raw.dtype == F32 and g.raw.dtype == F32 and u.raw.shape[0] >= u.rows and u.raw.shape[1] >= u.C
+    assert g.raw.shape[0] >= (g.B - 1) * g.bstride + g.n and g.raw.shape[1] >= g.C, "second source rows out of range"
+    d = H.AttpoolSrc()
+    d.U, d.ldu, d.G, d.ldg, d.g_bstride = u.raw.data_ptr(), u.raw.shape[1], g.raw.data_ptr(), g.raw.shape[1], g.bstride
+    if u.scale is not None:
+        d.u_scale, d.u_shift, d.u_act, d.u_slope = u.scale.data_ptr(), u.shift.data_ptr(), u.act, u.slope
+    if g.scale is not None:
+        d.g_scale, d.g_shift, d.g_act, d.g_slope = g.scale.data_ptr(), g.shift.data_ptr(), g.act, g.slope
+    assert u.n % 16 == 0
+    d.idx, d.n, d.h = idx.data_ptr(), u.n // 16, u.C
+    return d
+
+
+def attpool_concat_supported(x: ConcatGather, P: int, K: int) -> bool:
+    if not (x.u.raw.dtype == F32 and x.g.raw.dtype == F32 and x.u.bstride == x.u.n and x.u.C == x.g.C and x.u.n % 16 == 0):
+        return False
+    rc = H.lib().rl_attpool_cat_supported(C.byref(_attpool_src(x)), P, K, x.C)
+    if rc not in (0, H.ERR_UNSUPPORTED):
+        H.check(rc, "rl_attpool_cat_supported")
+    return rc == 0
+
+
+def attpool_fwd(X, S: torch.Tensor, P: int, K: int) -> torch.Tensor:
+    cat = isinstance(X, ConcatGather)
+    Cc = X.C if cat else X.shape[1]
+    assert S.shape == (P * K, Cc)
+    out = torch.empty((P, Cc), dtype=F32, device=S.device)
+    if cat:
+        src = _attpool_src(X)
+        _dev_check(S)
+        with _rec("attpool_fwd", (P, K, Cc), 4 * (P * K * X.u.C + X.g.rows * X.g.C + P * K + P * K * Cc + P * Cc), 0):
+            H.check(H.lib().rl_attpool_fwd_cat(C.byref(src), S.data_ptr(), P, K, Cc, out.data_ptr(), _st()), "rl_attpool_fwd_cat")
+        return out
     _dev_check(X, S)
-    Cc = X.shape[1]
-    assert X.shape == S.shape == (P * K, Cc)
-    out = torch.empty((P, Cc), dtype=F32, device=X.device)
+    assert X.shape == S.shape
     with _rec("attpool_fwd", (P, K, Cc), 4 * (2 * P * K * Cc + P * Cc), 0):
         H.check(H.lib().rl_attpool_fwd(X.data_ptr(), S.data_ptr(), P, K, Cc, out.data_ptr(), _st()), "rl_attpool_fwd")
     return out
 
 
 def attpool_bwd(X, S, Pout, dP, P: int, K: int):
-    _dev_check(X, S, Pout, dP)
-    Cc = X.shape[1]
-    assert X.shape == S.shape == (P * K, Cc) and Pout.shape == dP.shape == (P, Cc)
+    cat = isinstance(X, ConcatGather)
+    Cc = X.C if cat else X.shape[1]
+    _dev_check(S, Pout, dP)
+    assert S.shape == (P * K, Cc) and Pout.shape == dP.shape == (P, Cc)
     dS = torch.empty_like(S)
-    dXa = torch.empty_like(X)
+    dXa = torch.empty_like(S)
+    if cat:
+        src = _attpool_src(X)
+        with _rec("attpool_bwd", (P, K, Cc), 4 * (P * K * X.u.C + X.g.rows * X.g.C + P * K + 3 * P * K * Cc + 2 * P * Cc), 0):
+            H.check(H.lib().rl_attpool_bwd_cat(C.byref(src), S.data_ptr(), Pout.data_ptr(), dP.data_ptr(), P, K, Cc,
+                                               dS.data_ptr(), dXa.data_ptr(), _st()), "rl_attpool_bwd_cat")
+        return dS, dXa
+    _dev_check(X)
+    assert X.shape == S.shape and X.dtype == S.dtype
     with _rec("attpool_bwd", (P, K, Cc), 4 * (4 * P * K * Cc + 2 * P * Cc), 0):
         H.check(H.lib().rl_attpool_bwd(X.data_ptr(), S.data_ptr(), Pout.data_ptr(), dP.data_ptr(), P, K, Cc,
                                        dS.data_ptr(), dXa.data_ptr(), _st()), "rl_attpool_bwd")
diff --git a/include/rl_randlanet.h b/include/rl_randlanet.h
--- a/include/rl_randlanet.h
+++ b/include/rl_randlanet.h
@@ -91,9 +91,18 @@
     const float* bnb_invstd;
     int32_t bnb_act;
     float bnb_slope;
+    int32_t a2_split;
+    int32_t a2_act;
+    const float* A2;
+    int64_t lda2, a2_bstride;
+    const int32_t* a2_idx;
+    const float* a2_scale;
+    const float* a2_shift;
+    float a2_slope;
 } rl_gemm_desc;
 
 int rl_gemm_streams(const rl_gemm_desc* d);
+int rl_gemm_concat_supported(const rl_gemm_desc* d);
 int rl_gemm_pair_supported(const rl_gemm_desc* a, const rl_gemm_desc* b);
 int rl_gemm_pair(const rl_gemm_desc* a, const rl_gemm_desc* b, void* stream);
 
@@ -299,6 +308,30 @@
                    void* stream);
 int rl_attpool_bwd(const float* X, const float* S, const float* Pout, const float* dP, int64_t P,
                    int K, int C, float* dS, float* dXa, void* stream);
+
+typedef struct rl_attpool_src {
+    const float* U;
+    int64_t ldu;
+    const float* u_scale;
+    const float* u_shift;
+    int32_t u_act;
+    float u_slope;
+    const float* G;
+    int64_t ldg, g_bstride;
+    const float* g_scale;
+    const float* g_shift;
+    int32_t g_act;
+    float g_slope;
+    const int32_t* idx;
+    int32_t n;
+    int32_t h;
+} rl_attpool_src;
+int rl_attpool_cat_supported(const rl_attpool_src* x, int64_t P, int K, int C);
+int rl_attpool_fwd_cat(const rl_attpool_src* x, const float* S, int64_t P, int K, int C, float* Pout, void* stream);
+int rl_attpool_bwd_cat(const rl_attpool_src* x, const float* S, const float* Pout, const float* dP, int64_t P, int K, int C,
+                       float* dS, float* dXa, void* stream);
+int rl_set_pool256_x(const char* mode);
+const char* rl_get_pool256_x(void);
 
 typedef struct rl_pool_desc {
     const float* U;
```

Measured after the change: 1306 (median of 6 runs). 1.1% higher.
